# ElijahHyndman/PAPTeam_OpticalFlow

Hardware: AMD Instinct MI355X
Metric: Mpix/s per frame-pair (fixed SOR iters) at 1920x1080; max-abs d(u,v) vs ref (higher is better)
Workload: dtype f64

## Files before the change

papteam_opticalflow_amd/csrc/api.hip:

```cpp
#include <algorithm>
#include <chrono>
#include <cmath>
#include <cstdio>
#include <cstdlib>
#include <cstring>
#include <mutex>
#include <random>
#include <thread>

#include "common.h"
#include "flow_internal.h"

namespace papof {

namespace {
thread_local std::string g_last_error;
}

void set_last_error(const char* what, hipError_t e, const char* file, int line) {
    char buf[512];
    std::snprintf(buf, sizeof buf, "%s failed: %s (%s:%d)", what, hipGetErrorString(e), file, line);
    g_last_error = buf;
}
const char* last_error() { return g_last_error.c_str(); }
void set_last_error_text(const std::string& text) { g_last_error = text; }

static double wall() {
    return std::chrono::duration<double>(std::chrono::steady_clock::now().time_since_epoch()).count();
}

size_t arena_bytes_for(int H, int W, int C, int levels, int n_sor_max, double ratio) {
    const size_t np = (size_t)H * W;
    const int fc = (C == 3) ? 5 : (C == 1 ? 3 : C);
    size_t per_level = 0;
    {
        std::vector<Level> L;
        std::vector<PyrPlan> plan;
        if (levels >= 1 && pyramid_plan(H, W, ratio, levels, L, plan) == PAPOF_OK)
            for (const Level& l : L) per_level += ((size_t)l.w * l.h * fc * sizeof(double) + 256) * 3;
    }
    size_t sor_cells = 0, sor_cells_d = 0;
    skew_capacity(H, W, n_sor_max, sor_cells, sor_cells_d);
    size_t planes = 0;
    planes += (size_t)2 * C * 5;
    if (levels > 8) planes += (size_t)2 * C * levels;
    planes += (size_t)2 * C + 2 * C;
    planes += (size_t)7 * fc;
    planes += 8;
    planes += (size_t)3 * C + C;
    planes += (size_t)3 * fc;
    size_t bytes = planes * np * sizeof(double);
    bytes += 3 * (sor_cells + 2 * kLanes) * 16 + (sor_cells_d + 2 * kLanes) * 16 + 10 * np * sizeof(double);
    bytes += per_level + np * fc * sizeof(double);
    bytes += 8 * (std::min<size_t>(kTinyMaxCells, np) * sizeof(double) + 256);
    bytes += (size_t)64 * 4096;
    return bytes;
}

static size_t sor_scratch_bytes(int H, int W, int n_sor) {
    size_t cells = 0, cells_d = 0;
    skew_capacity(H, W, n_sor, cells, cells_d);
    return 4 * (cells + 128) * 16 + (cells_d + 128) * 16;
}

int ensure_arena(papof_handle* h, size_t bytes) {
    if (bytes <= h->arena.cap) return PAPOF_OK;
    PAPOF_HIP(hipStreamSynchronize(h->stream));
    if (h->arena.base) PAPOF_HIP(hipFree(h->arena.base));
    h->arena.base = nullptr;
    h->arena.cap = 0;
    void* p = nullptr;
    hipError_t e = hipMalloc(&p, bytes);
    if (e != hipSuccess) {
        set_last_error("hipMalloc(arena)", e, __FILE__, __LINE__);
        return PAPOF_ENOMEM;
    }
    h->arena.base = static_cast<char*>(p);
    h->arena.cap = bytes;
    return PAPOF_OK;
}

int check_params(const papof_params& P, int levels) {
    if (levels < 1) return PAPOF_EINVAL;
    if (P.n_inner < 1) return PAPOF_EINVAL;
    if (P.n_outer + 0 < 1 || P.n_sor < 1 || P.n_outer_per_level < 0 || P.n_sor_per_level < 0) return PAPOF_EINVAL;
    if (P.sor_mode < PAPOF_SOR_EXACT || P.sor_mode > PAPOF_SOR_JACOBI) return PAPOF_EINVAL;
    if (!(P.alpha > 0) || !(P.omega > 0)) return PAPOF_EINVAL;
    if (P.interpolation != PAPOF_INTERP_BILINEAR && P.interpolation != PAPOF_INTERP_BICUBIC) return PAPOF_EINVAL;
    if (P.noise_model != PAPOF_NOISE_LAPLACIAN && P.noise_model != PAPOF_NOISE_GMIXTURE) return PAPOF_EINVAL;
    return PAPOF_OK;
}

int pyramid_plan(int H, int W, double ratio, int nlev, std::vector<Level>& L, std::vector<PyrPlan>& plan) {
    ratio = effective_ratio(ratio);
    const double base_sigma = 1 / ratio - 1;
    const int n = (int)(std::log(0.25) / std::log(ratio));
    const double n_sigma = base_sigma * n;
    L.assign(nlev, Level{});
    plan.assign(nlev, PyrPlan{});
    L[0].w = W;
    L[0].h = H;
    for (int i = 1; i < nlev; i++) {
        PyrPlan p;
        if (i <= n) {
            p.src_level = 0;
            p.sigma = base_sigma * i;
            p.fsize = (int)(p.sigma * 3);
            p.rate = std::pow(ratio, i);
        } else {
            p.src_level = i - n;
            p.sigma = n_sigma;
            p.fsize = (int)(n_sigma * 3);
            p.rate = (double)std::pow(ratio, i) * W / L[i - n].w;
        }
        p.sw = L[p.src_level].w;
        p.sh = L[p.src_level].h;
        if (p.fsize > kMaxFsize) return PAPOF_EINVAL;
        L[i].w = (int)((double)p.sw * p.rate);
        L[i].h = (int)((double)p.sh * p.rate);
        if (L[i].w < 1 || L[i].h < 1) return PAPOF_EINVAL;
        plan[i] = p;
    }
    return PAPOF_OK;
}

papof_params params_or_default(const papof_params* params) {
    papof_params P;
    if (params)
        P = *params;
    else
        papof_default_params(&P);
    return P;
}

int call_plan(int H, int W, int C, int levels, const papof_params& P, CallPlan& cp) {
    PAPOF_TRY(check_params(P, levels));
    cp.ratio = effective_ratio(P.ratio);
    cp.levels = levels;
    cp.fc = feature_channels(C);
    PAPOF_TRY(pyramid_plan(H, W, P.ratio, levels, cp.L, cp.plan));
    cp.n_sor.resize(levels);
    cp.n_outer.resize(levels);
    for (int k = 0; k < levels; k++) {
        cp.n_sor[k] = CallPlan::n_sor_at(P, k);
        cp.n_outer[k] = CallPlan::n_outer_at(P, k);
    }
    cp.n_sor_max = cp.n_sor[levels - 1];
    cp.slots = CallPlan::slots_for(P, levels);
    cp.from_level0 = true;
    for (int i = 1; i < levels; i++) cp.from_level0 = cp.from_level0 && cp.plan[i].src_level == 0;
    return PAPOF_OK;
}

int lap_next_epoch(papof_handle* h, hipStream_t stream) {
    if (++h->lap_epoch >= kLapNone) {
        if (h->lap_flags_dev) PAPOF_HIP(hipMemsetAsync(h->lap_flags_dev, 0, kLapFlagWords * sizeof(unsigned), stream));
        h->lap_epoch = 1u;
    }
    return PAPOF_OK;
}

int fork_prep(papof_handle* h, int levels, bool overlap) {
    while (h->sync_events.size() < (size_t)levels + 2) {
        hipEvent_t e;
        PAPOF_HIP(hipEventCreateWithFlags(&e, hipEventDisableTiming));
        h->sync_events.push_back(e);
    }
    if (overlap) {
        PAPOF_HIP(hipEventRecord(h->sync_events[levels + 1], h->stream));
        PAPOF_HIP(hipStreamWaitEvent(h->prep_stream, h->sync_events[levels + 1], 0));
    }
    return PAPOF_OK;
}

int smooth_and_resize(papof_handle* h, const double* src, double* dst, double* tmp_a, double* tmp_b, const PyrPlan& p, int C,
                      int dh, int dw) {
    const Taps g = gaussian_taps(p.sigma, p.fsize);
    if (g.fsize == 0 && g.t[0] == 1.0) return resize(h, src, dst, p.sh, p.sw, C, dh, dw, p.rate, p.rate, false, 0.0);
    PAPOF_TRY(filter_hv(h, src, tmp_b, tmp_a, p.sh, p.sw, C, g, g));
    return resize(h, tmp_b, dst, p.sh, p.sw, C, dh, dw, p.rate, p.rate, false, 0.0);
}

int reduce_init(papof_handle* h, const papof_tensor* a, const papof_tensor* b, int pairs_a, int pairs_b, int H, int W,
                const std::vector<Level>& L, const std::vector<PyrPlan>& plan, double ratio, double* X, double* Y, double* T,
                size_t t_planes, double*& out) {
    const size_t np0 = (size_t)H * W;
    const int planes = 2 * (pairs_a + pairs_b), levels = (int)L.size();
    double* const parts[2] = {X, X + (size_t)pairs_a * 2 * np0};
    const papof_tensor* const src[2] = {a, b};
    const int n[2] = {pairs_a, pairs_b};
    for (int i = 0; i < 2; i++) {
        if (n[i] == 0) continue;
        if (src[i])
            PAPOF_TRY(ingest_frames(h, *src[i], nullptr, parts[i], H, W, 2, n[i]));
        else
            PAPOF_HIP(hipMemsetAsync(parts[i], 0, (size_t)n[i] * 2 * np0 * sizeof(double), h->stream));
    }
    PAPOF_TRY(init_sanitize(h, X, (size_t)planes * np0));
    out = X;
    if (levels == 1) return PAPOF_OK;
    std::vector<int> chain;
    for (int i = levels - 1; i > 0; i = plan[i].src_level) chain.insert(chain.begin(), i);
    double s = 1.0;
    for (int i = 1; i < levels; i++) s *= ratio;
    double *cur = X, *other = Y;
    for (const int i : chain) {
        const PyrPlan& p = plan[i];
        const bool last = i == levels - 1;
        const Taps g = gaussian_taps(p.sigma, p.fsize);
        if (g.fsize == 0 && g.t[0] == 1.0) {
            PAPOF_TRY(resize(h, cur, other, p.sh, p.sw, planes, L[i].h, L[i].w, p.rate, p.rate, last, last ? s : 0.0));
            std::swap(cur, other);
            continue;
        }
        const size_t ns = (size_t)p.sw * p.sh;
        const int chunk = filter_hv_needs_tmp(g, g) ? (int)std::min<size_t>((size_t)planes, t_planes * np0 / ns) : planes;
        if (chunk < 1) return PAPOF_EINVAL;
        for (int c0 = 0; c0 < planes; c0 += chunk)
            PAPOF_TRY(filter_hv(h, cur + c0 * ns, other + c0 * ns, T, p.sh, p.sw, std::min(chunk, planes - c0), g, g));
        PAPOF_TRY(resize(h, other, cur, p.sh, p.sw, planes, L[i].h, L[i].w, p.rate, p.rate, last, last ? s : 0.0));
    }
    out = cur;
    return PAPOF_OK;
}

int build_pyramid(papof_handle* h, const std::vector<Level>& L, const std::vector<PyrPlan>& plan, int C, bool second,
                  double* tmp_a, double* tmp_b) {
    for (size_t i = 1; i < L.size(); i++) {
        const PyrPlan& p = plan[i];
        const double* src = second ? L[p.src_level].p2 : L[p.src_level].p1;
        double* dst = second ? L[i].p2 : L[i].p1;
        PAPOF_TRY(smooth_and_resize(h, src, dst, tmp_a, tmp_b, p, C, L[i].h, L[i].w));
    }
    return PAPOF_OK;
}

struct SolveBuffers {
    double *im1s, *tmp, *blend, *imdt, *phi;
    SorPlanes sp;
    SorPlanes sp_tiny{};
    double *bgx = nullptr, *bgy = nullptr, *bgxy = nullptr;
    double *gm = nullptr, *gm_scratch = nullptr;
};

int alloc_solve_buffers(Arena& A, int H, int W, int fc, int mode, int n_sor_cap, SolveBuffers& B) {
    const size_t np = (size_t)H * W;
    B.im1s = A.f64(np * fc);
    B.tmp = A.f64(np * fc);
    B.blend = A.f64(np * fc);
    B.imdt = A.f64(np * fc);
    B.phi = A.f64(np);
    PAPOF_TRY(sor_alloc_planes(A, H, W, mode, n_sor_cap, B.sp));
    if (mode == PAPOF_SOR_EXACT)
        PAPOF_TRY(sor_alloc_tiny_planes(A, std::min<size_t>(kTinyMaxCells, (size_t)H * W), B.sp_tiny));
    return A.overflow ? PAPOF_ENOMEM : PAPOF_OK;
}

int alloc_branch_buffers(papof_handle* h, Arena& A, int H, int W, int fc, int interpolation, int noise_model,
                         SolveBuffers& B) {
    const size_t np = (size_t)H * W;
    if (interpolation == PAPOF_INTERP_BICUBIC) {
        B.bgx = A.f64(np * fc);
        B.bgy = A.f64(np * fc);
        B.bgxy = A.f64(np * fc);
    }
    if (noise_model == PAPOF_NOISE_GMIXTURE) {
        B.gm = A.f64(5 * 8);
        B.gm_scratch = A.f64((size_t)gm_scratch_doubles());
        if (A.overflow || fc > 8) return fc > 8 ? PAPOF_EINVAL : PAPOF_ENOMEM;
        double init[40];
        for (int k = 0; k < fc; k++) {
            init[k] = 0.95;
            init[fc + k] = 0.05;
            init[2 * fc + k] = 0.5;
            init[3 * fc + k] = 0.05 * 0.05;
            init[4 * fc + k] = 0.5 * 0.5;
        }
        PAPOF_HIP(hipMemcpyAsync(B.gm, init, sizeof(double) * 5 * fc, hipMemcpyHostToDevice, h->stream));
        PAPOF_HIP(hipStreamSynchronize(h->stream));
    }
    return A.overflow ? PAPOF_ENOMEM : PAPOF_OK;
}

struct LapGuard {
    bool on = false;
    bool exact = false;
    bool collect = false;
    bool nz_known = false;
    unsigned* flags = nullptr;
    double* lap = nullptr;
    double* scratch = nullptr;
    unsigned epoch = 0;
    int slot = 0;
    std::vector<int> slot_level, slot_channels;
    unsigned* wit(int s) const { return on && collect && s >= 0 && s < kLapMaxSlots ? flags + lap_wit_word(s) : nullptr; }
    unsigned* nz(int level) const { return on && collect && nz_known ? flags + lap_nz_word(level) : nullptr; }
    const double* guard() const { return on && exact ? lap : nullptr; }
    int unknown(const unsigned* host_flags) const {
        if (!on || !collect) return 0;
        if (slot > kLapMaxSlots) return 1;
        int n = 0;
        for (int s = 0; s + 1 < slot; s++)
            for (int c = 0; c < slot_channels[s]; c++) {
                const unsigned nz = host_flags[lap_nz_word(slot_level[s]) + c];
                const bool proven = lap_proven(host_flags[lap_wit_word(s) + c], epoch, nz_known, nz, nz);
                n += !proven;
                if (!proven && std::getenv("PAPOF_LAP_TRACE"))
                    std::fprintf(stderr, "[lap guard] no proof: slot %d of %d, level %d, channel %d\n", s, slot, slot_level[s], c);
            }
        return n;
    }
};

struct LevelSolve {
    SolveBuffers& B;
    const double *f1 = nullptr, *f2 = nullptr;
    double* warp = nullptr;
    int H = 0, W = 0, fc = 0;
    double alpha = 0, omega = 0;
    int n_outer = 0, n_inner = 0, n_sor = 0, mode = PAPOF_SOR_EXACT;
    const double* im1s_ready = nullptr;
    bool final_warp = true;
    const SolveCounters* counters = nullptr;
    double *out_u = nullptr, *out_v = nullptr;
    bool fold_warp = false;
    LapGuard* lg = nullptr;
    int level = 0;
};

static int marked_solve(papof_handle* h, PhaseClock& clk, unsigned* prog, SorPlanes& SP, const LevelSolve& s) {
    h->sor_mark = [](void* c, int on) {
        static_cast<PhaseClock*>(c)->phase(on ? PAPOF_T_PHASE5_SOR : PAPOF_T_PHASE6_UPDATE);
    };
    h->sor_mark_ctx = &clk;
    h->sor_prog_next = prog;
    const int rc = sor_solve(h, SP, s.H, s.W, s.alpha, s.omega, s.n_sor, s.mode);
    h->sor_prog_next = nullptr;
    h->sor_mark = nullptr;
    h->sor_mark_ctx = nullptr;
    return rc;
}

int smooth_flow(papof_handle* h, const LevelSolve& s, PhaseClock& clk, double*& u, double*& v, double*& ua, double*& va) {
    SolveBuffers& B = s.B;
    const Taps g = smooth5_taps();
    int solve_idx = 0;
    const bool tiny = s.mode == PAPOF_SOR_EXACT && B.sp_tiny.phi && sor_tiny_fits(h, s.H, s.W, s.n_sor);
    SorPlanes& SP = tiny ? B.sp_tiny : B.sp;
    const double* im1s = s.im1s_ready;
    if (!im1s) {
        clk.phase(PAPOF_T_PHASE1_GENERATE);
        PAPOF_TRY(filter_hv(h, s.f1, B.im1s, B.tmp, s.H, s.W, s.fc, g, g));
        im1s = B.im1s;
    }
    const char* const fused_sw = std::getenv("PAPOF_FUSED_SYSTEM");
    const bool fused_env = !(fused_sw && fused_sw[0] == '0');
    const bool fused_system = fused_env && s.fold_warp && s.n_inner == 1 && !B.gm && (s.fc == 5 || s.fc == 3) &&
                              !(s.lg && s.lg->guard()) && !(s.lg && s.lg->on && lap_one_block_level(s.H, s.W));
    for (int count = 0; count < s.n_outer; count++) {
        clk.phase(fused_system ? kTimerFused : (int)PAPOF_T_PHASE1_GENERATE);
        if (fused_system)
            PAPOF_TRY(flow_system(h, s.f1, s.f2, u, v, im1s, s.H, s.W, s.fc, s.alpha, s.omega, SP,
                                  s.lg && count > 0 ? s.lg->wit(s.lg->slot - 1) : nullptr));
        else if (s.fold_warp)
            PAPOF_TRY(warp_smooth_blend(h, s.f1, s.f2, u, v, im1s, B.blend, B.imdt, s.H, s.W, s.fc,
                                        s.lg && count > 0 && !B.gm ? s.lg->wit(s.lg->slot - 1) : nullptr,
                                        B.phi));
        else
            PAPOF_TRY(smooth_hv_blend(h, s.warp, im1s, B.blend, B.imdt, s.H, s.W, s.fc));
        for (int hh = 0; hh < s.n_inner; hh++) {
            const SorPlanes* prev = hh == 0 ? nullptr : &SP;
            if ((count == 0 && !s.fold_warp) || hh > 0) {
                clk.phase(PAPOF_T_PHASE2_DERIVATIVES);
                PAPOF_TRY(compute_phi(h, u, v, prev, B.phi, s.H, s.W));
            }
            if (!fused_system) clk.phase(PAPOF_T_PHASE4_LINEARSYSTEM);
            if (!fused_system)
                PAPOF_TRY(assemble_system(h, B.blend, B.imdt, B.phi, u, v, s.H, s.W, s.fc, s.alpha, s.omega, SP, nullptr, nullptr,
                                          prev, nullptr, B.gm, s.lg ? s.lg->guard() : nullptr));
            PAPOF_TRY(marked_solve(h, clk, s.counters ? s.counters->solve(h, s.level, (size_t)solve_idx) : nullptr, SP, s));
            solve_idx++;
        }
        double* const phi_next = count + 1 < s.n_outer && !s.fold_warp ? B.phi : nullptr;
        const bool rewarp = !s.fold_warp && !B.bgx && (s.final_warp || count + 1 < s.n_outer || B.gm);
        const bool wit_later = s.fold_warp && count + 1 < s.n_outer;
        const bool wit_small = s.fold_warp && !wit_later && lap_one_block_level(s.H, s.W);
        unsigned* const wit = s.lg && !B.gm && !B.bgx && !wit_later && !wit_small ? s.lg->wit(s.lg->slot) : nullptr;
        const bool to_caller = s.out_u && s.out_v && count + 1 == s.n_outer;
        PAPOF_TRY(update_warp_phi(h, SP, u, v, to_caller ? s.out_u : ua, to_caller ? s.out_v : va, s.f1, s.f2, s.warp, phi_next,
                                  s.H, s.W, s.fc, rewarp, 0, -1, wit));
        if (to_caller) {
            u = s.out_u;
            v = s.out_v;
        } else {
            std::swap(u, ua);
            std::swap(v, va);
        }
        if (B.bgx)
            PAPOF_TRY(bicubic_warp(h, s.f1, s.f2, B.bgx, B.bgy, B.bgxy, u, v, s.warp, s.H, s.W, s.fc, nullptr, true, true));
        if (s.lg && s.lg->on && !B.gm && wit_small && s.lg->wit(s.lg->slot))
            PAPOF_TRY(lap_small_check(h, s.f1, s.f2, u, v, s.H, s.W, s.fc, s.lg->wit(s.lg->slot)));
        if (s.lg && s.lg->on && !B.gm) {
            s.lg->slot_level.push_back(s.level);
            s.lg->slot_channels.push_back(s.fc);
            s.lg->slot++;
            if (s.lg->exact) {
                if (B.bgx)
                    PAPOF_TRY(est_laplacian_noise(h, s.f1, s.warp, nullptr, nullptr, s.H, s.W, s.fc, s.lg->lap, s.lg->scratch));
                else
                    PAPOF_TRY(est_laplacian_noise(h, s.f1, s.f2, u, v, s.H, s.W, s.fc, s.lg->lap, s.lg->scratch));
            }
        }
        if (B.gm) PAPOF_TRY(est_gaussian_mixture(h, s.f1, s.warp, s.H, s.W, s.fc, B.gm, B.gm_scratch));
    }
    clk.phase(-1);
    return PAPOF_OK;
}

int feature_channels(int C) { return C == 3 ? 5 : (C == 1 ? 3 : C); }

struct FrameIn {
    const void* d;
    bool u8;
    bool planar = false;
};
int load_frame(papof_handle* h, const FrameIn& f, double* planar, int H, int W, int C) {
    if (f.planar) {
        PAPOF_HIP(hipMemcpyAsync(planar, f.d, (size_t)H * W * C * sizeof(double), hipMemcpyDeviceToDevice, h->stream));
        return PAPOF_OK;
    }
    if (f.u8) return hwc_u8_to_planar(h, static_cast<const unsigned char*>(f.d), planar, H, W, C);
    return hwc_to_planar(h, static_cast<const double*>(f.d), planar, H, W, C);
}

enum SeqOp { kPair, kSeqPrime, kSeqNext };

bool seq_matches(const papof_handle* h, int H, int W, int C, int levels, double ratio, size_t need) {
    const papof_handle::Seq& q = h->seq;
    return q.valid && q.h == H && q.w == W && q.c == C && q.levels == levels && q.ratio == ratio &&
           q.arena_base == h->arena.base && need <= h->arena.cap;
}

struct FlowPass {
    papof_handle* h;
    const FrameIn &fa, &fb;
    SeqOp op;
    int H, W, C;
    const papof_params& P;
    double *d_vx, *d_vy, *d_warp;
    LapGuard* lg;
    const papof_tensor* init;
    CallPlan cp;
    int slot1 = 0;
    double *tmp_a = nullptr, *tmp_b = nullptr;
    std::vector<double*> F1, F2, S1;
    double *gx = nullptr, *gy = nullptr, *gxy = nullptr;
    double *prep_tmp = nullptr, *warp = nullptr;
    double *u = nullptr, *v = nullptr, *u2 = nullptr, *v2 = nullptr;
    SolveBuffers B;
    bool exact = false;
    SolveCounters counters;
    bool overlap = false;
    bool hostio = false;
    hipStream_t main_stream = nullptr, prep = nullptr;
    PhaseClock clk, pclk, total;
};

static void keep_seq(const FlowPass& S, int slot) {
    S.h->seq = {.valid = true, .h = S.H, .w = S.W, .c = S.C, .levels = S.cp.levels, .slot = slot, .ratio = S.cp.ratio,
                .arena_base = S.h->arena.base};
}

static void start_clocks(FlowPass& S) {
    papof_handle* h = S.h;
    S.clk = S.pclk = S.total = PhaseClock{h, true};
    S.clk.only_sor = S.pclk.only_sor = (!h->phase_events && S.P.phase_timing == 0) || S.P.phase_timing == 2;
    h->sor_launches = 0;
    h->sor_log.clear();
    S.clk.stamps = true;
    h->stamps_used = 0;
    h->next_stamp = nullptr;
    h->stamp_stream = h->stream;
    S.total.phase(PAPOF_T_TOTAL);
}

static int carve_pyramids(FlowPass& S) {
    Arena& A = S.h->arena;
    for (Level& l : S.cp.L) {
        double* slot[2];
        slot[0] = A.f64((size_t)l.w * l.h * S.C);
        slot[1] = A.f64((size_t)l.w * l.h * S.C);
        l.p1 = slot[S.slot1];
        l.p2 = slot[S.slot1 ^ 1];
    }
    const size_t np0 = (size_t)S.H * S.W;
    S.tmp_a = A.f64(np0 * S.C);
    S.tmp_b = A.f64(np0 * S.C);
    return A.overflow ? PAPOF_ENOMEM : PAPOF_OK;
}

static int carve_buffers(FlowPass& S) {
    papof_handle* h = S.h;
    Arena& A = h->arena;
    const CallPlan& cp = S.cp;
    const int levels = cp.levels, fc = cp.fc;
    const size_t np0 = (size_t)S.H * S.W;
    S.F1.resize(levels);
    S.F2.resize(levels);
    S.S1.resize(levels);
    for (int k = 0; k < levels; k++) {
        const size_t n = (size_t)cp.L[k].w * cp.L[k].h * fc;
        S.F1[k] = A.f64(n);
        S.F2[k] = A.f64(n);
        S.S1[k] = A.f64(n);
    }
    S.prep_tmp = A.f64(np0 * fc);
    S.gx = A.f64(np0 * S.C);
    S.gy = A.f64(np0 * S.C);
    S.gxy = A.f64(np0 * S.C);
    S.warp = A.f64(np0 * fc);
    S.u = A.f64(2 * np0);
    S.v = S.u ? S.u + np0 : nullptr;
    S.u2 = A.f64(2 * np0);
    S.v2 = S.u2 ? S.u2 + np0 : nullptr;
    PAPOF_TRY(alloc_solve_buffers(A, S.H, S.W, fc, S.P.sor_mode, cp.n_sor_max, S.B));
    PAPOF_TRY(alloc_branch_buffers(h, A, S.H, S.W, fc, S.P.interpolation, S.P.noise_model, S.B));
    S.exact = S.P.sor_mode == PAPOF_SOR_EXACT;
    if (S.exact) {
        S.counters = SolveCounters(cp, [&](int k) { return sor_counters_words(cp.L[k].h, cp.L[k].w, cp.n_sor[k]); },
                                   (size_t)S.P.n_inner);
        PAPOF_TRY(sor_counters_ensure(h, S.counters.total));
    }
    return PAPOF_OK;
}

static bool prep_kept(const FlowPass& S, int second) { return second == 0 && S.op == kSeqNext; }
static int prep_build_level(FlowPass& S, int i, int second) {
    if (i == 0 || prep_kept(S, second)) return PAPOF_OK;
    const std::vector<Level>& L = S.cp.L;
    const PyrPlan& q = S.cp.plan[i];
    const double* src = second ? L[q.src_level].p2 : L[q.src_level].p1;
    return smooth_and_resize(S.h, src, second ? L[i].p2 : L[i].p1, S.tmp_a, S.tmp_b, q, S.C, L[i].h, L[i].w);
}
static int prep_level_ready(FlowPass& S, int k) {
    S.pclk.phase(-1);
    if (S.overlap) PAPOF_HIP(hipEventRecord(S.h->sync_events[k], S.prep));
    return PAPOF_OK;
}
static int prep_frames(FlowPass& S, int first, int last, bool chained, bool smooth, bool ready) {
    const std::vector<Level>& L = S.cp.L;
    const int levels = S.cp.levels;
    const Taps g5 = smooth5_taps();
    S.pclk.phase(PAPOF_T_CONSTRUCTION);
    for (int second = first; second < last; second++)
        if (!prep_kept(S, second)) PAPOF_TRY(load_frame(S.h, second ? S.fb : S.fa, second ? L[0].p2 : L[0].p1, S.H, S.W, S.C));
    for (int i = 1; chained && i < levels; i++)
        for (int second = first; second < last; second++) PAPOF_TRY(prep_build_level(S, i, second));
    for (int k = levels - 1; k >= 0; k--) {
        if (!chained) {
            S.pclk.phase(PAPOF_T_CONSTRUCTION);
            for (int second = first; second < last; second++) PAPOF_TRY(prep_build_level(S, k, second));
        }
        S.pclk.phase(PAPOF_T_ALLOCATION);
        for (int second = first; second < last; second++)
            PAPOF_TRY(im2feature(S.h, second ? L[k].p2 : L[k].p1, second ? S.F2[k] : S.F1[k], L[k].h, L[k].w, S.C,
                                 S.lg ? S.lg->nz(k) : nullptr));
        if (smooth) {
            S.pclk.phase(PAPOF_T_PHASE1_GENERATE);
            PAPOF_TRY(filter_hv(S.h, S.F1[k], S.S1[k], S.prep_tmp, L[k].h, L[k].w, S.cp.fc, g5, g5));
        }
        if (ready) PAPOF_TRY(prep_level_ready(S, k));
    }
    return PAPOF_OK;
}
static int prep_final_planes(FlowPass& S) {
    S.pclk.phase(PAPOF_T_POSTPROCESSING);
    PAPOF_TRY(central3_planes(S.h, S.cp.L[0].p2, S.gx, S.gy, S.gxy, S.H, S.W, S.C));
    return prep_level_ready(S, S.cp.levels);
}
static int prep_upload(FlowPass& S, const void* host, const FrameIn& f, int event) {
    papof_handle* h = S.h;
    if (!host) return PAPOF_OK;
    PAPOF_HIP(hipMemcpyAsync(const_cast<void*>(f.d), host, h->hostio.nb_in, hipMemcpyHostToDevice, h->copy_stream));
    PAPOF_HIP(hipEventRecord(h->copy_events[event], h->copy_stream));
    PAPOF_HIP(hipStreamWaitEvent(S.prep, h->copy_events[event], 0));
    return PAPOF_OK;
}

static int prepare(FlowPass& S) {
    StreamSwap on_prep(S.h, S.prep);
    const bool chained = !S.cp.from_level0;
    S.pclk.phase(PAPOF_T_ALLOCATION);
    if (S.exact && !sor_counters_clear(S.h, 0, S.counters.total)) return PAPOF_EDEVICE;
    if (!S.hostio) {
        PAPOF_TRY(prep_frames(S, 0, 2, chained, true, true));
    } else {
        PAPOF_TRY(prep_upload(S, S.h->hostio.im1, S.fa, 0));
        PAPOF_TRY(prep_frames(S, 0, 1, true, true, false));
        S.pclk.phase(-1);
        PAPOF_TRY(prep_upload(S, S.h->hostio.im2, S.fb, 1));
        PAPOF_TRY(prep_frames(S, 1, 2, chained, false, true));
    }
    return prep_final_planes(S);
}

static int fork_and_prepare(FlowPass& S) {
    papof_handle* h = S.h;
    const papof_handle::HostIO& io = h->hostio;
    S.overlap = h->overlap_prep && S.P.phase_timing != 1 && h->prep_stream != nullptr;
    S.main_stream = h->stream;
    S.prep = S.overlap ? h->prep_stream : h->stream;
    S.hostio = io.active && S.overlap && h->copy_stream && h->copy_events.size() >= 8;
    if (io.active && !S.hostio) {
        if (io.im1) PAPOF_HIP(hipMemcpyAsync(const_cast<void*>(S.fa.d), io.im1, io.nb_in, hipMemcpyHostToDevice, S.main_stream));
        if (io.im2) PAPOF_HIP(hipMemcpyAsync(const_cast<void*>(S.fb.d), io.im2, io.nb_in, hipMemcpyHostToDevice, S.main_stream));
    }
    PAPOF_TRY(fork_prep(h, S.cp.levels, S.overlap));
    const int rc = prepare(S);
    if (rc != PAPOF_OK && S.overlap) hipStreamSynchronize(S.prep);
    return rc;
}

static int enter_level(FlowPass& S, int k, int pw, int ph, bool fold_warp) {
    papof_handle* h = S.h;
    const int lw = S.cp.L[k].w, lh = S.cp.L[k].h, fc = S.cp.fc;
    const size_t np = (size_t)lw * lh;
    const double *f1 = S.F1[k], *f2 = S.F2[k];
    SolveBuffers& B = S.B;
    const bool coarsest = k == S.cp.levels - 1;
    if (coarsest && S.init) {
        double* r = nullptr;
        PAPOF_TRY(reduce_init(h, S.init, nullptr, 1, 0, S.H, S.W, S.cp.L, S.cp.plan, S.cp.ratio, S.u, S.u2, S.warp, (size_t)fc, r));
        if (r != S.u) std::swap(S.u, S.u2);
    } else if (coarsest) {
        PAPOF_HIP(hipMemsetAsync(S.u, 0, 2 * np * sizeof(double), h->stream));
        if (!fold_warp) PAPOF_HIP(hipMemcpyAsync(S.warp, f2, np * fc * sizeof(double), hipMemcpyDeviceToDevice, h->stream));
    } else {
        PAPOF_TRY(resize(h, S.u, S.u2, ph, pw, 2, lh, lw, (double)lw / pw, (double)lh / ph, true, 1 / S.cp.ratio));
        std::swap(S.u, S.u2);
    }
    S.v = S.u + np;
    S.v2 = S.u2 + np;
    if (B.bgx) PAPOF_TRY(central3_planes(h, f2, B.bgx, B.bgy, B.bgxy, lh, lw, fc));
    if (coarsest && !S.init) return PAPOF_OK;
    if (B.bgx)
        PAPOF_TRY(bicubic_warp(h, f1, f2, B.bgx, B.bgy, B.bgxy, S.u, S.v, S.warp, lh, lw, fc, nullptr, true, false));
    else if (!fold_warp)
        PAPOF_TRY(warp_bilinear(h, f1, f2, S.u, S.v, S.warp, lh, lw, fc));
    return PAPOF_OK;
}

static int solve_levels(FlowPass& S) {
    papof_handle* h = S.h;
    const CallPlan& cp = S.cp;
    LapGuard* const lg = S.lg;
    if (lg && lg->guard())
        PAPOF_HIP(hipMemcpyAsync(lg->lap, h->lap_init_dev, 8 * sizeof(double), hipMemcpyDeviceToDevice, S.main_stream));
    int pw = 0, ph = 0;
    for (int k = cp.levels - 1; k >= 0; k--) {
        const int lw = cp.L[k].w, lh = cp.L[k].h;
        S.clk.phase(-1);
        if (S.overlap) PAPOF_HIP(hipStreamWaitEvent(S.main_stream, h->sync_events[k], 0));
        S.clk.phase(PAPOF_T_ALLOCATION);
        const bool tiny_k = S.exact && sor_tiny_fits(h, lh, lw, cp.n_sor[k]);
        if (!tiny_k) PAPOF_TRY(sor_bind(h, S.B.sp, lh, lw, cp.n_sor[k]));
        const LevelSolve s{.B = S.B, .f1 = S.F1[k], .f2 = S.F2[k], .warp = S.warp, .H = lh, .W = lw, .fc = cp.fc,
                           .alpha = S.P.alpha, .omega = S.P.omega, .n_outer = cp.n_outer[k], .n_inner = S.P.n_inner,
                           .n_sor = cp.n_sor[k], .mode = S.P.sor_mode, .im1s_ready = S.S1[k], .final_warp = false,
                           .counters = S.exact ? &S.counters : nullptr, .out_u = k == 0 ? S.d_vx : nullptr,
                           .out_v = k == 0 ? S.d_vy : nullptr, .fold_warp = !S.B.bgx && !S.B.gm, .lg = lg, .level = k};
        PAPOF_TRY(enter_level(S, k, pw, ph, s.fold_warp));
        if (!tiny_k) PAPOF_TRY(sor_reset_planes(h, S.B.sp));
        PAPOF_TRY(smooth_flow(h, s, S.clk, S.u, S.v, S.u2, S.v2));
        pw = lw;
        ph = lh;
    }
    return PAPOF_OK;
}

static int final_warp(FlowPass& S) {
    papof_handle* h = S.h;
    papof_handle::HostIO& io = h->hostio;
    const int H = S.H, W = S.W, C = S.C, levels = S.cp.levels;
    const size_t np0 = (size_t)H * W;
    const Level& l0 = S.cp.L[0];
    S.clk.phase(-1);
    if (S.overlap) PAPOF_HIP(hipStreamWaitEvent(S.main_stream, h->sync_events[levels], 0));
    S.clk.phase(PAPOF_T_POSTPROCESSING);
    if (S.hostio && io.early_out && S.u == S.d_vx && S.v == S.d_vy) {
        hipStream_t const cs = h->copy_stream;
        PAPOF_HIP(hipEventRecord(h->copy_events[2], S.main_stream));
        PAPOF_HIP(hipStreamWaitEvent(cs, h->copy_events[2], 0));
        PAPOF_HIP(hipMemcpyAsync(io.vx, S.d_vx, io.nb_flow, hipMemcpyDeviceToHost, cs));
        PAPOF_HIP(hipMemcpyAsync(io.vy, S.d_vy, io.nb_flow, hipMemcpyDeviceToHost, cs));
        constexpr int kChunks = 4;
        for (int q = 0; q < kChunks; q++) {
            const Rect rc{0, (int)((long long)H * q / kChunks), W, (int)((long long)H * (q + 1) / kChunks)};
            if (rc.empty()) continue;
            PAPOF_TRY(bicubic_warp(h, l0.p1, l0.p2, S.gx, S.gy, S.gxy, S.u, S.v, S.d_warp, H, W, C, &rc));
            PAPOF_HIP(hipEventRecord(h->copy_events[3 + q], S.main_stream));
            PAPOF_HIP(hipStreamWaitEvent(cs, h->copy_events[3 + q], 0));
            const size_t off = (size_t)rc.y0 * W * C, cnt = (size_t)rc.h() * W * C;
            PAPOF_HIP(hipMemcpyAsync(io.warp + off, S.d_warp + off, cnt * sizeof(double), hipMemcpyDeviceToHost, cs));
        }
        io.out_issued = true;
        return PAPOF_OK;
    }
    PAPOF_TRY(bicubic_warp(h, l0.p1, l0.p2, S.gx, S.gy, S.gxy, S.u, S.v, S.d_warp, H, W, C));
    if (S.u != S.d_vx) PAPOF_HIP(hipMemcpyAsync(S.d_vx, S.u, np0 * sizeof(double), hipMemcpyDeviceToDevice, h->stream));
    if (S.v != S.d_vy) PAPOF_HIP(hipMemcpyAsync(S.d_vy, S.v, np0 * sizeof(double), hipMemcpyDeviceToDevice, h->stream));
    return PAPOF_OK;
}

static int fetch_flags_and_stamps(FlowPass& S) {
    papof_handle* h = S.h;
    const LapGuard* lg = S.lg;
    h->stamps_fetched = 0;
    const bool flags = lg && lg->on && lg->collect;
    const size_t first = flags ? lap_wit_word(std::min(lg->slot, kLapMaxSlots) - 1) : kLapFlagWords;
    const size_t bytes = (kLapFlagWords - first) * sizeof(unsigned) + (size_t)h->stamps_used * sizeof(unsigned long long);
    if (bytes > 0)
        PAPOF_HIP(hipMemcpyAsync(h->lap_flags_host + first, h->lap_flags_dev + first, bytes, hipMemcpyDeviceToHost, h->stream));
    h->stamps_fetched = h->stamps_used;
    return PAPOF_OK;
}

static void report_timers(double* tm) {
    {
        constexpr double kPsiShare = 0.3;
        const double fused = tm[PAPOF_T_PHASE4_LINEARSYSTEM];
        tm[PAPOF_T_PHASE3_PSIDATA] += kPsiShare * fused;
        tm[PAPOF_T_PHASE4_LINEARSYSTEM] = fused - kPsiShare * fused;
    }
    {
        constexpr double kPhiShare = 0.04;
        const double fused = tm[PAPOF_T_PHASE1_GENERATE];
        tm[PAPOF_T_PHASE2_DERIVATIVES] += kPhiShare * fused;
        tm[PAPOF_T_PHASE1_GENERATE] = fused - kPhiShare * fused;
    }
    {
        const double f = tm[kTimerFused];
        tm[PAPOF_T_PHASE1_GENERATE] += 0.51 * f;
        tm[PAPOF_T_PHASE2_DERIVATIVES] += 0.02 * f;
        tm[PAPOF_T_PHASE3_PSIDATA] += 0.14 * f;
        tm[PAPOF_T_PHASE4_LINEARSYSTEM] += f - 0.51 * f - 0.02 * f - 0.14 * f;
    }
}

int flow_pass(papof_handle* h, const FrameIn& fa, const FrameIn& fb, SeqOp op, int H, int W, int C, int levels,
              const papof_params& P, double* d_vx, double* d_vy, double* d_warp, double* timing, LapGuard* lg,
              const papof_tensor* init = nullptr) {
    const double t_entry = wall();
    FlowPass S{h, fa, fb, op, H, W, C, P, d_vx, d_vy, d_warp, lg, init};
    PAPOF_TRY(call_plan(H, W, C, levels, P, S.cp));
    const size_t need = arena_bytes_for(H, W, C, levels, S.cp.n_sor_max, P.ratio);
    if (op == kSeqNext && !seq_matches(h, H, W, C, levels, S.cp.ratio, need)) {
        g_last_error = "sequence push does not continue the primed sequence (shape, levels, ratio or arena changed)";
        return PAPOF_EINVAL;
    }
    S.slot1 = op == kSeqNext ? h->seq.slot : 0;
    h->seq.valid = false;
    PAPOF_TRY(ensure_arena(h, need));
    h->arena.off = 0;
    h->arena.overflow = false;
    h->events_used = 0;
    double tm[PAPOF_N_TIMERS + 1];
    std::memset(tm, 0, sizeof tm);
    start_clocks(S);
    PAPOF_TRY(carve_pyramids(S));
    if (op == kSeqPrime) {
        PAPOF_TRY(load_frame(h, fa, S.cp.L[0].p1, H, W, C));
        PAPOF_TRY(build_pyramid(h, S.cp.L, S.cp.plan, C, false, S.tmp_a, S.tmp_b));
        PAPOF_HIP(hipStreamSynchronize(h->stream));
        keep_seq(S, S.slot1);
        if (timing) std::memset(timing, 0, PAPOF_N_TIMERS * sizeof(double));
        return PAPOF_OK;
    }
    PAPOF_TRY(carve_buffers(S));
    PAPOF_TRY(fork_and_prepare(S));
    int rc_main = solve_levels(S);
    if (rc_main == PAPOF_OK) rc_main = final_warp(S);
    if (rc_main != PAPOF_OK) {
        hipStreamSynchronize(S.main_stream);
        if (S.overlap) hipStreamSynchronize(S.prep);
        return rc_main;
    }
    S.clk.phase(-1);
    PAPOF_TRY(stamp_only(h));
    S.total.phase(-1);
    PAPOF_TRY(fetch_flags_and_stamps(S));
    const double t_enqueued = wall();
    PAPOF_HIP(hipStreamSynchronize(h->stream));
    h->host_enqueue_sec = t_enqueued - t_entry;
    h->host_wait_sec = wall() - t_enqueued;
    h->next_stamp = nullptr;
    if (S.exact) PAPOF_TRY(sor_check(h));
    if (S.clk.err != PAPOF_OK || S.pclk.err != PAPOF_OK || S.total.err != PAPOF_OK) return PAPOF_EDEVICE;
    S.clk.collect(tm);
    S.pclk.collect(tm);
    S.total.collect(tm);
    if (S.clk.sor_span_sec.size() == h->sor_log.size())
        for (size_t i = 0; i < h->sor_log.size(); i++) h->sor_log[i].sec = S.clk.sor_span_sec[i];
    report_timers(tm);
    if (timing) std::memcpy(timing, tm, PAPOF_N_TIMERS * sizeof(double));
    if (op == kSeqNext) keep_seq(S, S.slot1 ^ 1);
    return PAPOF_OK;
}

int flow_device(papof_handle* h, const FrameIn& fa, const FrameIn& fb, SeqOp op, int H, int W, int C, int levels,
                const papof_params& P, double* d_vx, double* d_vy, double* d_warp, double* timing,
                const papof_tensor* init = nullptr) {
    LapGuard lg;
    const int fc = feature_channels(C);
    lg.on = h->lap_guard && op != kSeqPrime && P.noise_model == PAPOF_NOISE_LAPLACIAN && fc <= 8 && levels >= 1 &&
            h->lap_flags_dev != nullptr;
    if (!lg.on) return flow_pass(h, fa, fb, op, H, W, C, levels, P, d_vx, d_vy, d_warp, timing, nullptr, init);
    lg.flags = h->lap_flags_dev;
    lg.lap = h->lap_dev;
    lg.scratch = h->lap_scratch_dev;
    lg.nz_known = (C == 1 || C == 3) && (size_t)levels * 8 <= (size_t)kLapNzWords;
    const bool always_exact = P.interpolation == PAPOF_INTERP_BICUBIC;
    lg.collect = !always_exact;
    lg.exact = always_exact || h->lap_exact;
    const papof_handle::Seq seq0 = h->seq;
    double first_pass_total = 0.0;
    for (int pass = 0; pass < 2; pass++) {
        PAPOF_TRY(lap_next_epoch(h, h->stream));
        lg.epoch = h->lap_epoch;
        lg.slot = 0;
        lg.slot_level.clear();
        lg.slot_channels.clear();
        PAPOF_TRY(flow_pass(h, fa, fb, op, H, W, C, levels, P, d_vx, d_vy, d_warp, timing, &lg, init));
        if (pass == 1 && timing) timing[PAPOF_T_TOTAL] += first_pass_total;
        if (!lg.collect) return PAPOF_OK;
        const int unknown = lg.unknown(h->lap_flags_host);
        if (lg.exact) {
            if (pass == 0) h->lap_exact_calls++;
            h->lap_exact = unknown > 0;
            return PAPOF_OK;
        }
        if (unknown == 0) return PAPOF_OK;
        h->lap_reruns++;
        lg.exact = true;
        if (timing) first_pass_total = timing[PAPOF_T_TOTAL];
        if (h->copy_stream) PAPOF_HIP(hipStreamSynchronize(h->copy_stream));
        h->seq = seq0;
        h->hostio.im1 = nullptr;
        h->hostio.im2 = nullptr;
    }
    return PAPOF_OK;
}

int flow_device_planar(papof_handle* h, const double* f1, const double* f2, int H, int W, int C, int levels,
                       const papof_params& P, double* d_vx, double* d_vy, double* d_warp, double* timing,
                       const papof_tensor* init) {
    FrameIn a{f1, false}, b{f2, false};
    a.planar = b.planar = true;
    return flow_device(h, a, b, kPair, H, W, C, levels, P, d_vx, d_vy, d_warp, timing, init);
}

}
// ... 653 lines not shown
    PAPOF_TRY(S.down_planar(sp.b1, rhs1, height, width, 1));
    return S.down_planar(sp.b2, rhs2, height, width, 1);
}

int papof_stage_laplacian(papof_handle* h, const double* in, const double* weight, int height, int width,
                          double* out) {
    if (!h || !in || !weight || !out || height < 1 || width < 1) return PAPOF_EINVAL;
    Scope S(h, img_bytes(height, width, 1, 6));
    PAPOF_TRY(S.rc);
    double* a = S.up_planar(in, height, width, 1);
    double* w = S.up_planar(weight, height, width, 1);
    double* o = S.dev((size_t)height * width);
    PAPOF_TRY(S.rc);
    PAPOF_TRY(laplacian(h, a, w, o, height, width));
    return S.down_planar(o, out, height, width, 1);
}

namespace {
int alloc_sor_planes(Scope& S, int H, int W, int mode, int n_sor, SorPlanes& sp) {
    if (mode == PAPOF_SOR_EXACT && sor_tiny_fits(S.h, H, W, n_sor)) {
        const int rc_t = sor_alloc_tiny_planes(S.h->arena, (size_t)H * W, sp);
        if (rc_t != PAPOF_OK) S.rc = rc_t;
        return S.rc;
    }
    int rc = sor_alloc_planes(S.h->arena, H, W, mode, n_sor, sp);
    if (rc == PAPOF_OK) rc = sor_bind(S.h, sp, H, W, n_sor);
    if (rc != PAPOF_OK) S.rc = rc;
    return S.rc;
}
}

int papof_stage_sor(papof_handle* h, const double* phi, const double* imdxy, const double* imdx2,
                    const double* imdy2, const double* rhs1, const double* rhs2, int height, int width,
                    double alpha, double omega, int n_sor, int sor_mode, double* du, double* dv) {
    if (!h || !phi || !imdxy || !imdx2 || !imdy2 || !rhs1 || !rhs2 || !du || !dv || height < 1 || width < 1 ||
        n_sor < 1 || sor_mode < PAPOF_SOR_EXACT || sor_mode > PAPOF_SOR_JACOBI)
        return PAPOF_EINVAL;
    const size_t np = (size_t)height * width;
    Scope S(h, img_bytes(height, width, 1, 16) + sor_scratch_bytes(height, width, n_sor) +
                   12 * (size_t)height * width * sizeof(double));
    PAPOF_TRY(S.rc);
    double* p = S.up_planar(phi, height, width, 1);
    double* xy = S.up_planar(imdxy, height, width, 1);
    double* x2 = S.up_planar(imdx2, height, width, 1);
    double* y2 = S.up_planar(imdy2, height, width, 1);
    double* r1 = S.up_planar(rhs1, height, width, 1);
    double* r2 = S.up_planar(rhs2, height, width, 1);
    double *ou = S.dev(np), *ov = S.dev(np);
    SorPlanes sp{};
    PAPOF_TRY(alloc_sor_planes(S, height, width, sor_mode, n_sor, sp));
    PAPOF_TRY(sor_reset_planes(h, sp));
    PAPOF_TRY(sor_prep(h, p, xy, x2, y2, r1, r2, height, width, alpha, omega, sp));
    PAPOF_TRY(sor_solve(h, sp, height, width, alpha, omega, n_sor, sor_mode));
    PAPOF_TRY(sor_unpack(h, sp, ou, ov, height, width));
    PAPOF_TRY(S.down_planar(ou, du, height, width, 1));
    PAPOF_TRY(S.down_planar(ov, dv, height, width, 1));
    if (sor_mode == PAPOF_SOR_EXACT) PAPOF_TRY(sor_check(h));
    return PAPOF_OK;
}

int papof_stage_smoothflow(papof_handle* h, const double* im1, const double* im2, double* warp, double* u,
                           double* v, int height, int width, int c, double alpha, int n_outer, int n_inner,
                           int n_sor, double omega, int sor_mode) {
    return papof_stage_smoothflow_ex(h, im1, im2, warp, u, v, height, width, c, alpha, n_outer, n_inner, n_sor, omega,
                                     sor_mode, PAPOF_INTERP_BILINEAR, PAPOF_NOISE_LAPLACIAN, nullptr);
}

int papof_stage_smoothflow_ex(papof_handle* h, const double* im1, const double* im2, double* warp, double* u,
                              double* v, int height, int width, int c, double alpha, int n_outer, int n_inner,
                              int n_sor, double omega, int sor_mode, int interpolation, int noise_model, double* gm) {
    if (!h || !im1 || !im2 || !warp || !u || !v || height < 1 || width < 1 || c < 1 || n_outer < 1 || n_sor < 1 ||
        sor_mode < PAPOF_SOR_EXACT || sor_mode > PAPOF_SOR_JACOBI)
        return PAPOF_EINVAL;
    if (n_inner < 1) return PAPOF_EINVAL;
    if (interpolation < 0 || interpolation > 1 || noise_model < 0 || noise_model > 1) return PAPOF_EINVAL;
    Scope S(h, img_bytes(height, width, c, 16) + img_bytes(height, width, 1, 8) +
                   sor_scratch_bytes(height, width, n_sor) +
                   12 * (size_t)height * width * sizeof(double) + (1 << 20));
    PAPOF_TRY(S.rc);
    double* f1 = S.up_planar(im1, height, width, c);
    double* f2 = S.up_planar(im2, height, width, c);
    double* w = S.up_planar(warp, height, width, c);
    double* du = S.up_planar(u, height, width, 1);
    double* dv = S.up_planar(v, height, width, 1);
    double* du_alt = S.dev((size_t)height * width);
    double* dv_alt = S.dev((size_t)height * width);
    PAPOF_TRY(S.rc);
    SolveBuffers B;
    PAPOF_TRY(alloc_solve_buffers(h->arena, height, width, c, sor_mode, n_sor, B));
    PAPOF_TRY(alloc_branch_buffers(h, h->arena, height, width, c, interpolation, noise_model, B));
    if (B.gm && gm) PAPOF_HIP(hipMemcpyAsync(B.gm, gm, sizeof(double) * 5 * c, hipMemcpyHostToDevice, h->stream));
    if (B.bgx) PAPOF_TRY(central3_planes(h, f2, B.bgx, B.bgy, B.bgxy, height, width, c));
    PAPOF_TRY(sor_bind(h, B.sp, height, width, n_sor));
    PAPOF_TRY(sor_reset_planes(h, B.sp));
    PhaseClock clk{h, false};
    LapGuard lg;
    lg.on = h->lap_guard && noise_model == PAPOF_NOISE_LAPLACIAN && c <= 8 && h->lap_dev != nullptr;
    lg.exact = true;
    lg.lap = h->lap_dev;
    lg.scratch = h->lap_scratch_dev;
    if (lg.on) PAPOF_HIP(hipMemcpyAsync(lg.lap, h->lap_init_dev, 8 * sizeof(double), hipMemcpyDeviceToDevice, h->stream));
    const LevelSolve s{.B = B, .f1 = f1, .f2 = f2, .warp = w, .H = height, .W = width, .fc = c, .alpha = alpha, .omega = omega,
                       .n_outer = n_outer, .n_inner = n_inner, .n_sor = n_sor, .mode = sor_mode, .lg = &lg};
    PAPOF_TRY(smooth_flow(h, s, clk, du, dv, du_alt, dv_alt));
    PAPOF_TRY(S.down_planar(w, warp, height, width, c));
    PAPOF_TRY(S.down_planar(du, u, height, width, 1));
    PAPOF_TRY(S.down_planar(dv, v, height, width, 1));
    if (B.gm && gm) {
        PAPOF_HIP(hipMemcpyAsync(gm, B.gm, sizeof(double) * 5 * c, hipMemcpyDeviceToHost, h->stream));
        PAPOF_HIP(hipStreamSynchronize(h->stream));
    }
    if (sor_mode == PAPOF_SOR_EXACT) PAPOF_TRY(sor_check(h));
    return PAPOF_OK;
}

int papof_stage_est_gaussian_mixture(papof_handle* h, const double* im1, const double* im2, int height, int width,
                                     int c, double* gm) {
    if (!h || !im1 || !im2 || !gm || height < 1 || width < 1 || c < 1 || c > 8) return PAPOF_EINVAL;
    Scope S(h, img_bytes(height, width, c, 6) + (1 << 20));
    PAPOF_TRY(S.rc);
    double* a = S.up_planar(im1, height, width, c);
    double* b = S.up_planar(im2, height, width, c);
    double* g = S.dev(40);
    double* scratch = S.dev((size_t)gm_scratch_doubles());
    PAPOF_TRY(S.rc);
    PAPOF_HIP(hipMemcpyAsync(g, gm, sizeof(double) * 5 * c, hipMemcpyHostToDevice, h->stream));
    PAPOF_TRY(est_gaussian_mixture(h, a, b, height, width, c, g, scratch));
    PAPOF_HIP(hipMemcpyAsync(gm, g, sizeof(double) * 5 * c, hipMemcpyDeviceToHost, h->stream));
    PAPOF_HIP(hipStreamSynchronize(h->stream));
    return PAPOF_OK;
}

int papof_pyramid_levels_for_min_width(int width, double ratio, int min_width, int* levels) {
    if (width < 1 || min_width < 1 || !levels) return PAPOF_EINVAL;
    ratio = effective_ratio(ratio);
    *levels = (int)(std::log((double)min_width / width) / std::log(ratio));
    return PAPOF_OK;
}

int papof_sor_tiny_shape(int height, int width, int* cells_per_tile, int* waves) {
    if (height < 1 || width < 1 || !cells_per_tile || !waves) return PAPOF_EINVAL;
    sor_tiny_shape(height, width, cells_per_tile, waves);
    return PAPOF_OK;
}

int papof_stage_bicubic_warp(papof_handle* h, const double* im1, const double* im2, const double* vx,
                             const double* vy, int height, int width, int c, double* out) {
    return papof_stage_bicubic_warp_ex(h, im1, im2, vx, vy, height, width, c, 1, out);
}

int papof_stage_bicubic_warp_ex(papof_handle* h, const double* im1, const double* im2, const double* vx,
                                const double* vy, int height, int width, int c, int clamp, double* out) {
    if (!h || !im1 || !im2 || !vx || !vy || !out || height < 1 || width < 1 || c < 1) return PAPOF_EINVAL;
    Scope S(h, img_bytes(height, width, c, 10) + img_bytes(height, width, 1, 4));
    PAPOF_TRY(S.rc);
    const size_t n = (size_t)height * width * c;
    double* a = S.up_planar(im1, height, width, c);
    double* b = S.up_planar(im2, height, width, c);
    double* fx = S.up_planar(vx, height, width, 1);
    double* fy = S.up_planar(vy, height, width, 1);
    double *gx = S.dev(n), *gy = S.dev(n), *gxy = S.dev(n), *o = S.dev(n);
    PAPOF_TRY(S.rc);
    PAPOF_TRY(central3_planes(h, b, gx, gy, gxy, height, width, c));
    PAPOF_TRY(bicubic_warp(h, a, b, gx, gy, gxy, fx, fy, o, height, width, c, nullptr, false, clamp != 0));
    PAPOF_HIP(hipMemcpyAsync(out, o, n * sizeof(double), hipMemcpyDeviceToHost, h->stream));
    PAPOF_HIP(hipStreamSynchronize(h->stream));
    return PAPOF_OK;
}

int papof_flow_quantize16(papof_handle* h, const double* vx, const double* vy, int height, int width,
                          unsigned short* out) {
    if (!h || !vx || !vy || !out || height < 1 || width < 1) return PAPOF_EINVAL;
    const size_t n = (size_t)height * width;
    Scope S(h, n * (2 * sizeof(double) + 2 * sizeof(unsigned short)) + 4096);
    PAPOF_TRY(S.rc);
    double* a = S.up_planar(vx, height, width, 1);
    double* b = S.up_planar(vy, height, width, 1);
    unsigned short* q = reinterpret_cast<unsigned short*>(S.dev((n * 2 * sizeof(unsigned short) + 7) / 8));
    PAPOF_TRY(S.rc);
    PAPOF_TRY(flow_quantize16(h, a, b, q, n));
    PAPOF_HIP(hipMemcpyAsync(out, q, n * 2 * sizeof(unsigned short), hipMemcpyDeviceToHost, h->stream));
    PAPOF_HIP(hipStreamSynchronize(h->stream));
    return PAPOF_OK;
}

int papof_flow_dequantize16(papof_handle* h, const unsigned short* q, int height, int width, double* vx,
                            double* vy) {
    if (!h || !q || !vx || !vy || height < 1 || width < 1) return PAPOF_EINVAL;
    const size_t n = (size_t)height * width;
    Scope S(h, n * (2 * sizeof(double) + 2 * sizeof(unsigned short)) + 4096);
    PAPOF_TRY(S.rc);
    unsigned short* dq = reinterpret_cast<unsigned short*>(S.dev((n * 2 * sizeof(unsigned short) + 7) / 8));
    double* a = S.dev(n);
    double* b = S.dev(n);
    PAPOF_TRY(S.rc);
    PAPOF_HIP(hipMemcpyAsync(dq, q, n * 2 * sizeof(unsigned short), hipMemcpyHostToDevice, h->stream));
    PAPOF_TRY(flow_dequantize16(h, dq, a, b, n));
    PAPOF_HIP(hipMemcpyAsync(vx, a, n * sizeof(double), hipMemcpyDeviceToHost, h->stream));
    PAPOF_HIP(hipMemcpyAsync(vy, b, n * sizeof(double), hipMemcpyDeviceToHost, h->stream));
    PAPOF_HIP(hipStreamSynchronize(h->stream));
    return PAPOF_OK;
}

int papof_flow_to_bgr(papof_handle* h, const double* vx, const double* vy, int height, int width,
                      unsigned char* bgr) {
    if (!h || !vx || !vy || !bgr || height < 1 || width < 1) return PAPOF_EINVAL;
    const size_t n = (size_t)height * width;
    Scope S(h, n * (2 * sizeof(double) + 3) + 16384);
    PAPOF_TRY(S.rc);
    double* a = S.up_planar(vx, height, width, 1);
    double* b = S.up_planar(vy, height, width, 1);
    double* partial = S.dev(512);
    unsigned char* out = reinterpret_cast<unsigned char*>(S.dev((n * 3 + 7) / 8));
    PAPOF_TRY(S.rc);
    PAPOF_TRY(flow_to_bgr(h, a, b, n, partial, out));
    PAPOF_HIP(hipMemcpyAsync(bgr, out, n * 3, hipMemcpyDeviceToHost, h->stream));
    PAPOF_HIP(hipStreamSynchronize(h->stream));
    return PAPOF_OK;
}

int papof_sor_plan(papof_handle* h, int height, int width, int n_sor, int sor_mode, int* launches, int* depth) {
    return sor_plan(h, height, width, n_sor, sor_mode, launches, depth);
}

int papof_last_sor_stats(papof_handle* h, int* launches, double* strip_streams_sec) {
    if (!h) return PAPOF_EINVAL;
    if (launches) *launches = h->sor_launches;
    if (strip_streams_sec) *strip_streams_sec = 0.0;
    return PAPOF_OK;
}

int papof_lap_guard_stats(papof_handle* h, int out[4]) {
    if (!h || !out) return PAPOF_EINVAL;
    out[0] = h->lap_reruns;
    out[1] = h->lap_exact_calls;
    out[2] = h->lap_exact ? 1 : 0;
    out[3] = h->lap_guard ? 1 : 0;
    return PAPOF_OK;
}

int papof_last_host_times(papof_handle* h, double out[3]) {
    if (!h || !out) return PAPOF_EINVAL;
    out[0] = h->host_enqueue_sec;
    out[1] = h->host_wait_sec;
    out[2] = 0.0;
    return PAPOF_OK;
}

int papof_last_sor_solves(papof_handle* h, int cap, int* n, int* info, double* sec) {
    if (!h || !n) return PAPOF_EINVAL;
    *n = (int)h->sor_log.size();
    for (int i = 0; i < *n && i < cap; i++) {
        const papof_handle::SorSolveLog& e = h->sor_log[i];
        if (info) {
            int* o = info + (size_t)i * 6;
            o[0] = e.H;
            o[1] = e.W;
            o[2] = e.n_sor;
            o[3] = e.kind;
            o[4] = e.depth;
            o[5] = e.launches;
        }
        if (sec) sec[i] = e.sec;
    }
    return PAPOF_OK;
}

int papof_test_sor_strips(papof_handle* h, int height, int width, int n_sor, int split_band, int reps, int delay_us,
                          long long* mismatches, int* bands) {
    if (!h || !mismatches) return PAPOF_EINVAL;
    const size_t np = (size_t)height * width;
    Scope S(h, img_bytes(height, width, 1, 16) + sor_scratch_bytes(height, width, n_sor) +
                   12 * (size_t)height * width * sizeof(double));
    PAPOF_TRY(S.rc);
    std::vector<double> host(np * 6);
    std::mt19937_64 rng(2);
    auto fill = [&](size_t k, double lo, double hi) {
        std::uniform_real_distribution<double> d(lo, hi);
        for (size_t i = 0; i < np; i++) host[k * np + i] = d(rng);
    };
    fill(0, 0.5, 50.0);
    fill(1, -0.02, 0.02);
    fill(2, 0.0, 0.05);
    fill(3, 0.0, 0.05);
    fill(4, -0.01, 0.01);
    fill(5, -0.01, 0.01);
    double* planes[6];
    for (int k = 0; k < 6; k++) planes[k] = S.up_planar(host.data() + k * np, height, width, 1);
    SorPlanes sp{};
    PAPOF_TRY(alloc_sor_planes(S, height, width, PAPOF_SOR_EXACT, n_sor, sp));
    PAPOF_TRY(sor_reset_planes(h, sp));
    PAPOF_TRY(sor_prep(h, planes[0], planes[1], planes[2], planes[3], planes[4], planes[5], height, width, 0.012, 1.8, sp));
    if (bands) *bands = sp.sd.nb;
    const size_t cells = sp.sd.nd;
    std::vector<double> want(cells * 2), got(cells * 2);
    PAPOF_TRY(sor_solve(h, sp, height, width, 0.012, 1.8, n_sor, PAPOF_SOR_EXACT));
    PAPOF_HIP(hipStreamSynchronize(h->stream));
    PAPOF_TRY(sor_check(h));
    PAPOF_HIP(hipMemcpy(want.data(), sp.du, cells * 16, hipMemcpyDeviceToHost));
    *mismatches = 0;
    if (!sor_strips_supported(h, sp, n_sor) || split_band < 1 || split_band >= sp.sd.nb) return PAPOF_EINVAL;
    struct Owned {
        hipStream_t top = nullptr;
        hipEvent_t ev = nullptr;
        ~Owned() {
            if (top) {
                hipStreamSynchronize(top);
                hipStreamDestroy(top);
            }
            if (ev) hipEventDestroy(ev);
        }
    } own;
    PAPOF_HIP(hipStreamCreateWithFlags(&own.top, hipStreamNonBlocking));
    PAPOF_HIP(hipEventCreateWithFlags(&own.ev, hipEventDisableTiming));
    hipStream_t const main_stream = h->stream, top = own.top;
    hipEvent_t const ev = own.ev;
    for (int r = 0; r < reps; r++) {
// ... 172 lines not shown
```

papteam_opticalflow_amd/csrc/common.h:

```cpp
#pragma once
#include <cstdlib>

#include <hip/hip_runtime.h>

#include <algorithm>
#include <cmath>
#include <cstddef>
#include <cstdint>
#include <initializer_list>
#include <string>
#include <vector>

#include "../../include/papof.h"

namespace papof {

constexpr int kLanes = 64;
constexpr int kMaxFsize = 8;

struct Rect {
    int x0, y0, x1, y1;
    __host__ __device__ bool empty() const { return x1 <= x0 || y1 <= y0; }
    __host__ __device__ int w() const { return x1 - x0; }
    __host__ __device__ int h() const { return y1 - y0; }
// ... 114 lines not shown
        d.hp = (d.rt + kBandRows * d.nb + 2 + 7) / 8 * 8;
        d.npos = d.qt + d.ns + 2 * kSorMaxDepth + 2 + kBandRows * (d.nb - 1) + 2;
        d.dpar = d.group == 1 ? ((n_sor - 1) & 1) : (((n_sor + d.group - 1) / d.group - 1) & 1);
        d.koff = n_sor - 1;
        d.poff = 1;
        d.nh = d.group == 1 ? 0 : (size_t)n_sor * d.nb * d.npos_d;
    }
    d.n = (size_t)d.npos * d.hp;
    d.nd = (size_t)2 * d.npos_d * d.nb * kLanes;
    return d;
}
inline void skew_capacity(int h, int w, int n_sor, size_t& cells, size_t& cells_d) {
    const SkewDims a = skew_dims(h, w, n_sor, 2), b = skew_dims(h, w, n_sor, 1, 2);
    cells = a.n > b.n ? a.n : b.n;
    cells_d = (a.nd + a.nh) > (b.nd + b.nh) ? (a.nd + a.nh) : (b.nd + b.nh);
}

struct SorPlanes {
    double *phi, *xy, *a1, *a2, *b1, *b2;
    double *du, *dv;
    double *du2, *dv2;
    bool skew;
    SkewDims sd;
    size_t cap_cells, cap_cells_d;
};

}

struct papof_handle {
    int device = 0;
    hipStream_t stream = nullptr;
    papof::Arena arena;
    unsigned* sync_words = nullptr;
    size_t sync_cap = 0;
    std::vector<hipEvent_t> events;
    size_t events_used = 0;
    int cu_count = 0;
    double* stage_dev = nullptr;
    size_t stage_dev_bytes = 0;
    double* tensor_scratch = nullptr;
    size_t tensor_scratch_bytes = 0;
    hipEvent_t entry_event = nullptr;
    unsigned* init_flag_dev = nullptr;
    bool use_dpp = false;
    int sor_depth = 0;
    unsigned long long* sor_dbg = nullptr;
    void (*sor_mark)(void*, int) = nullptr;
    void* sor_mark_ctx = nullptr;
    int sor_fuse = 0;
    int sor_group = 0;
    int rb_depth = 0;
    int rb_shape = 0;
    int sor_tiny = 1;
    int sor_resident = 0;
    int sor_skip_dead = 1;
    unsigned* sor_prog_next = nullptr;
    int sor_launches = 0;
    struct SorSolveLog {
        int H, W, n_sor, kind, depth, launches;
        double sec;
    };
    std::vector<SorSolveLog> sor_log;
    hipStream_t prep_stream = nullptr;
    unsigned* lap_flags_dev = nullptr;
    unsigned* lap_flags_host = nullptr;
    double* lap_dev = nullptr;
    double* lap_init_dev = nullptr;
    double* lap_scratch_dev = nullptr;
    bool lap_guard = true;
    bool lap_exact = false;
    unsigned lap_epoch = 0;
    int lap_reruns = 0, lap_exact_calls = 0;
    long long batch_chains = 0, batch_chain_pairs = 0, batch_singles = 0, batch_reruns = 0;
    double host_enqueue_sec = 0.0, host_wait_sec = 0.0;
    struct HostIO {
        bool active = false;
        const void *im1 = nullptr, *im2 = nullptr;
        size_t nb_in = 0;
        double *vx = nullptr, *vy = nullptr, *warp = nullptr;
        size_t nb_flow = 0, nb_img = 0;
        bool early_out = false;
        bool out_issued = false;
    } hostio;
    hipStream_t copy_stream = nullptr;
    std::vector<hipEvent_t> copy_events;
    std::vector<hipEvent_t> sync_events;
    bool overlap_prep = true;
    unsigned long long* stamps_dev = nullptr;
    unsigned long long* stamps = nullptr;
    int stamps_cap = 0, stamps_used = 0, stamps_fetched = 0;
    unsigned long long* next_stamp = nullptr;
    hipStream_t stamp_stream = nullptr;
    bool phase_events = true;
    int sor_xcd_affine = 1;
    struct Seq {
        bool valid = false;
        int h = 0, w = 0, c = 0, levels = 0, slot = 0;
        double ratio = 0;
        const char* arena_base = nullptr;
    } seq;
};

namespace papof {

inline unsigned long long* take_stamp(papof_handle* h) {
    if (h->stamp_stream && h->stream != h->stamp_stream) return nullptr;
    unsigned long long* s = h->next_stamp;
    h->next_stamp = nullptr;
    return s;
}
int stamp_only(papof_handle* h);

inline bool described(const papof_tensor* t, std::initializer_list<int> dtypes, std::initializer_list<int> axes, bool positive) {
    if (!t || !t->data || std::find(dtypes.begin(), dtypes.end(), t->dtype) == dtypes.end()) return false;
    for (int i : axes)
        if (t->stride[i] < 0 || (positive && t->stride[i] == 0)) return false;
    return true;
}
constexpr std::initializer_list<int> kImageDtypes = {PAPOF_DTYPE_U8, PAPOF_DTYPE_F32, PAPOF_DTYPE_F64};
constexpr std::initializer_list<int> kFlowDtypes = {PAPOF_DTYPE_F32, PAPOF_DTYPE_F64};
inline bool in_frames(const papof_tensor* t) { return described(t, kImageDtypes, {0, 1, 2, 3}, false); }
inline bool out_frames(const papof_tensor* t) { return described(t, kImageDtypes, {0, 1, 2, 3}, true); }
inline bool in_flow(const papof_tensor* t) { return described(t, kFlowDtypes, {0, 1, 2, 3}, false); }
inline bool out_flow(const papof_tensor* t) { return described(t, kFlowDtypes, {0, 1, 2, 3}, true); }
inline bool in_flow_pair(const papof_tensor* fw, const papof_tensor* bw) { return in_flow(fw) && in_flow(bw); }
inline bool opt_in_mask(const papof_tensor* t) { return !t || described(t, {PAPOF_DTYPE_U8}, {0, 1, 2}, false); }
inline bool opt_out_mask(const papof_tensor* t) { return !t || described(t, {PAPOF_DTYPE_U8}, {0, 1, 2}, true); }
inline bool opt_in_plane(const papof_tensor* t) { return !t || described(t, kFlowDtypes, {0, 1, 2}, false); }
inline bool opt_out_plane(const papof_tensor* t) { return !t || described(t, kFlowDtypes, {0, 1, 2}, true); }
inline bool valid_alphas(double a1, double a2) { return std::isfinite(a1) && std::isfinite(a2) && a1 >= 0 && a2 >= 0; }
inline long long dtype_bytes(int dtype) { return dtype == PAPOF_DTYPE_U8 ? 1 : dtype == PAPOF_DTYPE_F32 ? 4 : 8; }

int hwc_to_planar(papof_handle* h, const double* hwc, double* planar, int H, int W, int C, int frames = 1);
int hwc_u8_to_planar(papof_handle* h, const unsigned char* hwc, double* planar, int H, int W, int C, int frames = 1);
int planar_to_hwc(papof_handle* h, const double* planar, double* hwc, int H, int W, int C);
int ingest_frames(papof_handle* h, const papof_tensor& a, const papof_tensor* b, double* planar, int H, int W, int C,
                  int frames);
int emit_outputs(papof_handle* h, const double* src, const papof_tensor& dst, bool comp_major, int H, int W, int K, int pairs);
int init_check(papof_handle* h, const papof_tensor& t, int pairs, int H, int W, unsigned* flag);
int init_sanitize(papof_handle* h, double* planar, size_t n);
int fb_check(papof_handle* h, hipStream_t st, const papof_tensor& fw, const papof_tensor& bw, const papof_tensor& mask,
             int pairs, int H, int W, double a1, double a2);
int filter_h(papof_handle* h, const double* src, double* dst, int H, int W, int planes, const Taps& f,
             const Rect* rc = nullptr);
int filter_v(papof_handle* h, const double* src, double* dst, int H, int W, int planes, const Taps& f,
             const Rect* rc = nullptr);
int filter_hv(papof_handle* h, const double* src, double* dst, double* tmp, int H, int W, int planes, const Taps& fh,
              const Taps& fv);
bool filter_hv_needs_tmp(const Taps& fh, const Taps& fv);
int resize(papof_handle* h, const double* src, double* dst, int sh, int sw, int planes, int dh, int dw, double xr,
           double yr, bool use_post, double post, const Rect* rc = nullptr);
int im2feature(papof_handle* h, const double* im, double* feat, int H, int W, int C, unsigned* nz = nullptr, int frames = 1,
               size_t nz_stride = 0);
int central3_planes(papof_handle* h, const double* src, double* gx, double* gy, double* gxy, int H, int W, int planes);
int warp_bilinear(papof_handle* h, const double* im1, const double* im2, const double* vx, const double* vy,
                  double* out, int H, int W, int planes, const Rect* rc = nullptr);
int smooth_v_blend(papof_handle* h, const double* tmp, const double* im1s, double* blend, double* imdt, int H,
                   int W, int planes, const Rect* rc = nullptr);
int smooth_hv_blend(papof_handle* h, const double* warp, const double* im1s, double* blend, double* imdt, int H,
                    int W, int planes, int row0 = 0, int row1 = -1);
int warp_smooth_blend(papof_handle* h, const double* im1, const double* im2, const double* u, const double* v,
                      const double* im1s, double* blend, double* imdt, int H, int W, int planes, unsigned* wit = nullptr,
                      double* phi_out = nullptr);
int compute_phi(papof_handle* h, const double* u, const double* v, const SorPlanes* prev, double* phi, int H, int W,
                const Rect* rc = nullptr);
int assemble_system(papof_handle* h, const double* blend, const double* imdt, const double* phi, const double* u,
                    const double* v, int H, int W, int planes, double alpha, double omega, const SorPlanes& out,
                    double* opt_imdx2, double* opt_imdy2, const SorPlanes* prev, const Rect* rc = nullptr,
                    const double* gm = nullptr, const double* lap = nullptr);
int flow_system(papof_handle* h, const double* im1, const double* im2, const double* u, const double* v, const double* im1s,
                int H, int W, int planes, double alpha, double omega, const SorPlanes& out, unsigned* wit = nullptr,
                int row0 = 0, int row1 = -1,
                int batch = 1, const BatchK* bk = nullptr);
int lap_scratch_doubles();
int lap_rows_check(papof_handle* h, const double* im1, const double* im2, const double* u, const double* v, int H, int W,
                   int C, int r0, int r1, unsigned* wit, unsigned* val, unsigned mark);
bool lap_one_block_level(int H, int W);
int lap_small_check(papof_handle* h, const double* im1, const double* im2, const double* u, const double* v, int H, int W,
                    int C, unsigned* wit, int batch = 1, const BatchK* bk = nullptr);
int est_laplacian_noise(papof_handle* h, const double* im1, const double* im2, const double* u, const double* v, int H,
                        int W, int C, double* lap, double* scratch);
int gm_scratch_doubles();
int est_gaussian_mixture(papof_handle* h, const double* im1, const double* im2, int H, int W, int C, double* gm,
                         double* scratch);
int laplacian(papof_handle* h, const double* in, const double* weight, double* out, int H, int W);
int bicubic_warp(papof_handle* h, const double* im1, const double* im2, const double* gx, const double* gy,
                 const double* gxy, const double* vx, const double* vy, double* out_hwc, int H, int W, int C,
                 const Rect* rc = nullptr, bool planar_out = false, bool clamp = true, int batch = 1, const BatchK* bk = nullptr);
int flow_quantize16(papof_handle* h, const double* vx, const double* vy, unsigned short* q, size_t n);
int flow_dequantize16(papof_handle* h, const unsigned short* q, double* vx, double* vy, size_t n);
int flow_to_bgr(papof_handle* h, const double* vx, const double* vy, size_t n, double* partial, unsigned char* bgr);
int update_warp_phi(papof_handle* h, const SorPlanes& sp, const double* u, const double* v, double* u_out, double* v_out,
                    const double* im1, const double* im2, double* warp, double* phi_out, int H, int W, int planes,
                    bool do_warp = true, int row0 = 0, int row1 = -1, unsigned* wit = nullptr, int batch = 1,
                    const BatchK* bk = nullptr);
int update_flow(papof_handle* h, const SorPlanes& sp, double* u, double* v, int H, int W, const Rect& r);
int sor_prep(papof_handle* h, const double* phi, const double* imdxy, const double* imdx2, const double* imdy2,
             const double* rhs1, const double* rhs2, int H, int W, double alpha, double omega, const SorPlanes& out);
int sor_unpack(papof_handle* h, const SorPlanes& sp, double* du, double* dv, int H, int W);
Taps gaussian_taps(double sigma, int fsize);
Taps smooth5_taps();
Taps deriv5_taps();
Taps central3_taps();

struct SorBatch {
    int n;
    size_t coef, d, prog, tiny;
};
int sor_solve(papof_handle* h, const SorPlanes& sp, int H, int W, double alpha, double omega, int n_sor, int mode,
              const SorBatch* bt = nullptr);
int sor_blocked_depth(const papof_handle* h, int mode, int H, int W);
int sor_blocked_launch(papof_handle* h, const SorPlanes& sp, int H, int W, double alpha, double omega, int mode, int g,
                       int hs0, const Rect& out, const double* su, const double* sv, double* du, double* dv);
int sor_plan(const papof_handle* h, int H, int W, int n_sor, int mode, int* launches, int* depth);
int sor_check(papof_handle* h);
bool sor_strips_supported(const papof_handle* h, const SorPlanes& sp, int n_sor);
int sor_strips_begin(papof_handle* h, const SorPlanes& sp, int n_sor, int n_solves);
struct SorSplit {
    double* peer_du;
    unsigned* peer_prog;
    bool top_cut, bot_cut;
};
int sor_solve_bands(papof_handle* h, const SorPlanes& sp, int H, int W, double alpha, double omega, int n_sor,
                    unsigned* prog, int b0, int b1, const SorSplit* split = nullptr);
int sor_bind_plain(papof_handle* h, SorPlanes& sp, int H, int W, int n_sor);
constexpr size_t kTinyMaxCells = 8192;
bool sor_tiny_fits(const papof_handle* h, int H, int W, int n_sor);
bool sor_tiny_shape(int H, int W, int* cells_per_tile, int* waves);
int sor_alloc_tiny_planes(Arena& A, size_t cells, SorPlanes& sp);
size_t sor_counters_words(int H, int W, int n_sor);
int sor_counters_ensure(papof_handle* h, size_t words);
unsigned* sor_counters_clear(papof_handle* h, size_t offset_words, size_t words);
int sor_alloc_planes(Arena& A, int H, int W, int mode, int n_sor_cap, SorPlanes& sp);
int sor_bind(papof_handle* h, SorPlanes& sp, int H, int W, int n_sor);
int sor_group_size(const papof_handle* h, int H, int W, int n_sor);
int sor_reset_planes(papof_handle* h, const SorPlanes& sp);
int sor_reset_planes_batch(papof_handle* h, const SorPlanes& sp, int batch, size_t stride);
int sor_probe_dpp(papof_handle* h);

}
```

papteam_opticalflow_amd/csrc/flow_internal.h:

```cpp
#pragma once

#include <string>
#include <utility>
#include <vector>

#include "common.h"

namespace papof {

void set_last_error_text(const std::string& text);

constexpr int kTimerFused = PAPOF_N_TIMERS;
struct PhaseClock {
    papof_handle* h;
    bool on;
    std::vector<std::pair<int, std::pair<size_t, size_t>>> spans;
    size_t open = 0;
    int open_idx = -1;
    int err = PAPOF_OK;
    bool only_sor = false;
    bool stamps = false;
    std::vector<std::pair<int, int>> marks;
    std::vector<double> sor_span_sec;
    std::vector<int> sor_owner;
    size_t new_event() {
        if (h->events_used == h->events.size()) {
            hipEvent_t e;
            if (hipEventCreate(&e) != hipSuccess) {
                err = PAPOF_EDEVICE;
                return 0;
            }
            h->events.push_back(e);
        }
        hipEventRecord(h->events[h->events_used], h->stream);
        return h->events_used++;
    }
    void phase(int idx) {
        if (!on) return;
        if (stamps) {
            if (open_idx == PAPOF_T_PHASE5_SOR) {
                const size_t e = new_event();
                spans.push_back({PAPOF_T_PHASE5_SOR, {open, e}});
            }
            if (idx == PAPOF_T_PHASE5_SOR) {
                open = new_event();
                sor_owner.push_back(marks.empty() ? PAPOF_T_PHASE4_LINEARSYSTEM : marks.back().second);
            }
            const bool sor_edge = idx == PAPOF_T_PHASE5_SOR;
            open_idx = idx;
            if (only_sor || !h->stamps_dev || sor_edge) return;
            if (h->next_stamp && !marks.empty()) {
                marks.back().second = idx;
            } else if (h->stamps_used < h->stamps_cap) {
                const int slot = h->stamps_used++;
                h->next_stamp = h->stamps_dev + slot;
                marks.push_back({slot, idx});
            }
            return;
        }
        if (only_sor && idx != PAPOF_T_PHASE5_SOR && idx != PAPOF_T_TOTAL) {
            if (open_idx < 0) return;
            idx = -1;
        }
        const size_t e = new_event();
        if (open_idx >= 0) spans.push_back({open_idx, {open, e}});
        open = e;
        open_idx = idx;
    }
    void collect(double* t) {
        if (!on) return;
        for (auto& s : spans) {
            float ms = 0;
            if (hipEventElapsedTime(&ms, h->events[s.second.first], h->events[s.second.second]) == hipSuccess)
                t[s.first] += ms * 1e-3;
            if (s.first == PAPOF_T_PHASE5_SOR) sor_span_sec.push_back(ms * 1e-3);
        }
        for (size_t i = 0; i + 1 < marks.size(); i++) {
            const int idx = marks[i].second;
            if (marks[i + 1].first >= h->stamps_fetched) break;
            const unsigned long long a = h->stamps[marks[i].first], b = h->stamps[marks[i + 1].first];
            if (idx >= 0 && idx != PAPOF_T_PHASE5_SOR && b >= a) t[idx] += (double)(b - a) * 1e-8;
        }
        if (stamps && !marks.empty()) {
            for (size_t i = 0; i < sor_span_sec.size() && i < sor_owner.size(); i++)
                if (sor_owner[i] >= 0) t[sor_owner[i]] -= sor_span_sec[i];
            for (int own : {(int)PAPOF_T_PHASE4_LINEARSYSTEM, kTimerFused})
                if (t[own] < 0.0) t[own] = 0.0;
        }
    }
};

inline bool lap_proven(unsigned wit, unsigned epoch, bool nz_known, unsigned nz_a, unsigned nz_b) {
    const bool witness = wit == epoch || wit == (epoch ^ kLapNone);
    const bool all_zero = nz_known && nz_a != epoch && nz_b != epoch;
    return witness || all_zero;
}

struct Level {
    int w, h;
    double *p1, *p2;
};
struct PyrPlan {
    int sw, sh, src_level, fsize;
    double sigma, rate;
};

inline double effective_ratio(double ratio) { return ratio > 0.98 || ratio < 0.4 ? 0.75 : ratio; }
papof_params params_or_default(const papof_params* params);
struct CallPlan {
    double ratio = 0.75;
    int levels = 0, fc = 0;
    std::vector<Level> L;
    std::vector<PyrPlan> plan;
    std::vector<int> n_sor, n_outer;
    int n_sor_max = 0;
    long slots = 0;
    bool from_level0 = true;
    static int n_sor_at(const papof_params& P, int k) { return P.n_sor + k * P.n_sor_per_level; }
    static int n_outer_at(const papof_params& P, int k) { return P.n_outer + k * P.n_outer_per_level; }
    static long slots_for(const papof_params& P, int levels) {
        long s = 0;
        for (int k = 0; k < levels; k++) s += n_outer_at(P, k);
        return s;
    }
};
int call_plan(int H, int W, int C, int levels, const papof_params& P, CallPlan& cp);

inline unsigned* counters_base(const papof_handle* h) { return h->sync_words + 32; }
struct SolveCounters {
    struct PerLevel {
        size_t off = 0, per = 0;
    };
    std::vector<PerLevel> lv;
    size_t total = 0;
    SolveCounters() = default;
    template <class Words>
    SolveCounters(const CallPlan& cp, Words words, size_t solves_per_outer) : lv(cp.levels) {
        for (int k = 0; k < cp.levels; k++) {
            lv[k].per = words(k);
            lv[k].off = total;
            total += lv[k].per * (size_t)cp.n_outer[k] * solves_per_outer;
        }
    }
    unsigned* solve(const papof_handle* h, int k, size_t i) const { return counters_base(h) + lv[k].off + i * lv[k].per; }
};

int lap_next_epoch(papof_handle* h, hipStream_t stream);

inline int collect_total_and_sor(PhaseClock& total, PhaseClock& sorclk, double* timing) {
    if (total.err != PAPOF_OK || sorclk.err != PAPOF_OK) return PAPOF_EDEVICE;
    double tm[PAPOF_N_TIMERS + 1] = {};
    sorclk.collect(tm);
    total.collect(tm);
    for (int i = 0; timing && i < PAPOF_N_TIMERS; i++) timing[i] = tm[i];
    return PAPOF_OK;
}

struct StreamSwap {
    papof_handle* h;
    hipStream_t saved;
    StreamSwap(papof_handle* hh, hipStream_t s) : h(hh), saved(hh->stream) { h->stream = s; }
    ~StreamSwap() { h->stream = saved; }
};
int fork_prep(papof_handle* h, int levels, bool overlap);

size_t arena_bytes_for(int H, int W, int C, int levels, int n_sor_max, double ratio);
int ensure_arena(papof_handle* h, size_t bytes);
int check_params(const papof_params& P, int levels);
int pyramid_plan(int H, int W, double ratio, int nlev, std::vector<Level>& L, std::vector<PyrPlan>& plan);
int build_pyramid(papof_handle* h, const std::vector<Level>& L, const std::vector<PyrPlan>& plan, int C, bool second,
                  double* tmp_a, double* tmp_b);
int smooth_and_resize(papof_handle* h, const double* src, double* dst, double* tmp_a, double* tmp_b, const PyrPlan& p, int C,
                      int dh, int dw);
int feature_channels(int C);
int flow_batch_host(papof_handle* h, int n_pairs, int sequence, const void* const* frames, bool u8, int H, int W, int C, int levels,
                    const papof_params* params, double* const* vx, double* const* vy, double* const* warpI2, double* timing_sec);
int flow_device_planar(papof_handle* h, const double* f1, const double* f2, int H, int W, int C, int levels,
                       const papof_params& P, double* d_vx, double* d_vy, double* d_warp, double* timing,
                       const papof_tensor* init = nullptr);
int reduce_init(papof_handle* h, const papof_tensor* a, const papof_tensor* b, int pairs_a, int pairs_b, int H, int W,
                const std::vector<Level>& L, const std::vector<PyrPlan>& plan, double ratio, double* X, double* Y, double* T,
                size_t t_planes, double*& out);

}
```

papteam_opticalflow_amd/csrc/kernels.hip:

```cpp
#include "common.h"
#include "sampler.h"

#include <cmath>
#include <type_traits>

namespace papof {

namespace {

constexpr int BX = 64, BY = 4;

constexpr int tiles_of(int n, int t) { return (n + t - 1) / t; }
inline dim3 grid2d(int W, int H, int planes = 1) { return dim3(tiles_of(W, BX), tiles_of(H, BY), planes); }
inline Rect region(const Rect* rc, int W, int H) { return rc ? *rc : Rect{0, 0, W, H}; }
inline dim3 grid2d(const Rect& r, int planes = 1) { return grid2d(r.x1 - r.x0, r.y1 - r.y0, planes); }

__device__ __forceinline__ void stamp_now(unsigned long long* s) {
    if (s && (blockIdx.x | blockIdx.y | blockIdx.z | threadIdx.x | threadIdx.y) == 0u) *s = __builtin_amdgcn_s_memrealtime();
}
__global__ void k_stamp(unsigned long long* s) { stamp_now(s); }

__device__ __forceinline__ int clampi(int x, int n) {
    x = x < 0 ? 0 : x;
    return x > n - 1 ? n - 1 : x;
}

__device__ __forceinline__ bool xcd_tile(int ntx, int nty, int& tx, int& ty) {
    const int ntiles = ntx * nty, per = (ntiles + 7) >> 3;
    const int vt = (int)(blockIdx.x & 7u) * per + (int)(blockIdx.x >> 3);
    if ((int)(blockIdx.x >> 3) >= per || vt >= ntiles) return false;
    ty = vt / ntx;
    tx = vt - ty * ntx;
    return true;
}
static inline unsigned xcd_grid(int ntx, int nty) { return 8u * (unsigned)(((size_t)ntx * nty + 7) / 8); }

template <int HALF = -1, class At>
__device__ __forceinline__ double tap_sum(const Taps& f, At at, int half_rt = HALF) {
    const int half = HALF >= 0 ? HALF : half_rt;
    double acc = 0.0;
#pragma unroll
    for (int l = -half; l <= half; l++) acc += at(l) * f.t[l + half];
    return acc;
}

__device__ __forceinline__ void blend_imdt(double s1, double s2, double& blend, double& imdt) {
    double t = s1;
    t *= 0.4;
    t += s2 * 0.6;
    blend = t;
    imdt = s2 - s1;
}

__device__ __forceinline__ double phi_value(double uc, double vc, double ur, double vr, double ud, double vd, bool right,
                                            bool down) {
    const double ux = right ? ur - uc : 0.0;
    const double uy = down ? ud - uc : 0.0;
    const double vx = right ? vr - vc : 0.0;
    const double vy = down ? vd - vc : 0.0;
    const double t = ux * ux + uy * uy + vx * vx + vy * vy;
    return 0.5 / sqrt(t + 0.001 * 0.001);
}
__device__ __forceinline__ double phi_at(const double* __restrict__ u, const double* __restrict__ v, int i, int j, int H,
                                         int W) {
    const size_t o = (size_t)i * W + j;
    const double uc = u[o], vc = v[o];
    double ur = 0.0, vr = 0.0, ud = 0.0, vd = 0.0;
    if (j < W - 1) {
        ur = u[o + 1];
        vr = v[o + 1];
    }
    if (i < H - 1) {
        ud = u[o + W];
        vd = v[o + W];
    }
    return phi_value(uc, vc, ur, vr, ud, vd, j < W - 1, i < H - 1);
}

__device__ __forceinline__ bool leaves_image(double x, double y, int W, int H) {
    return x < 0 || x > W - 1 || y < 0 || y > H - 1;
}
__device__ __forceinline__ double bilinear_inside(double g0, double g1, double g2, double g3, double dx, double dy) {
    const double ex = 1.0 - dx, ey = 1.0 - dy;
    double res = 0.0;
    res += g0 * (ex * ey);
    res += g1 * (ex * dy);
    res += g2 * (dx * ey);
    res += g3 * (dx * dy);
    return res;
}
__device__ __forceinline__ double bilinear_inside_at(const double* __restrict__ p, int W, int H, double x, double y) {
    const int x0 = (int)x, y0 = (int)y;
    const int x1 = min(x0 + 1, W - 1), y1 = min(y0 + 1, H - 1);
    return bilinear_inside(p[y0 * W + x0], p[y1 * W + x0], p[y0 * W + x1], p[y1 * W + x1], x - x0, y - y0);
}

__device__ __forceinline__ bool lap_valid(double d) { return d > 0 && d < 1000000; }
__device__ __forceinline__ bool lap_witness(double d, double thr, bool sampled = true) {
    return sampled && d >= thr && d < 1000000;
}
__device__ __forceinline__ bool lap_one_in_sixteen(int tbx, int tby) { return ((tbx + 5 * tby) & 15) == 0; }
__device__ __forceinline__ bool lap_samples_here(int nblocks, int tbx, int tby) {
    return nblocks <= 256 || lap_one_in_sixteen(tbx, tby);
}

__global__ void k_hwc_to_planar(const double* __restrict__ hwc, double* __restrict__ planar, int H, int W, int C) {
    const int j = blockIdx.x * BX + threadIdx.x, i = blockIdx.y * BY + threadIdx.y;
    if (j >= W || i >= H) return;
    const size_t o = (size_t)i * W + j, np = (size_t)H * W;
    hwc += blockIdx.z * np * C;
    planar += blockIdx.z * np * C;
    for (int k = 0; k < C; k++) planar[k * np + o] = hwc[o * C + k];
}

__global__ void k_hwc_u8_to_planar(const unsigned char* __restrict__ hwc, double* __restrict__ planar, int H, int W,
                                   int C) {
    const int j = blockIdx.x * BX + threadIdx.x, i = blockIdx.y * BY + threadIdx.y;
    if (j >= W || i >= H) return;
    const size_t o = (size_t)i * W + j, np = (size_t)H * W;
    hwc += blockIdx.z * np * C;
    planar += blockIdx.z * np * C;
    for (int k = 0; k < C; k++) planar[k * np + o] = (double)hwc[o * C + k] / 255.0;
}

__global__ void k_planar_to_hwc(const double* __restrict__ planar, double* __restrict__ hwc, int H, int W, int C) {
    const int j = blockIdx.x * BX + threadIdx.x, i = blockIdx.y * BY + threadIdx.y;
    if (j >= W || i >= H) return;
    const size_t o = (size_t)i * W + j, np = (size_t)H * W;
    for (int k = 0; k < C; k++) hwc[o * C + k] = planar[k * np + o];
}

__device__ __forceinline__ double tensor_load(const void* p, int dtype, long long o) {
    if (dtype == PAPOF_DTYPE_U8) return (double)static_cast<const unsigned char*>(p)[o] / 255.0;
    if (dtype == PAPOF_DTYPE_F32) return (double)static_cast<const float*>(p)[o];
    return static_cast<const double*>(p)[o];
}

__global__ __launch_bounds__(256) void k_ingest_frames(const papof_tensor a, const papof_tensor b, int pairs,
                                                       double* __restrict__ planar, long long H, long long W, long long C,
                                                       long long total) {
    const long long i = (long long)blockIdx.x * blockDim.x + threadIdx.x;
    if (i >= total) return;
    const long long np = H * W, f = i / (np * C), r = i - f * np * C, c = r / np, px = r - c * np, row = px / W,
                    col = px - row * W;
    const bool second = pairs && (f & 1);
    const long long fi = pairs ? f >> 1 : f;
    const long long o = fi * (second ? b.stride[0] : a.stride[0]) + row * (second ? b.stride[1] : a.stride[1]) +
                        col * (second ? b.stride[2] : a.stride[2]) + c * (second ? b.stride[3] : a.stride[3]);
    planar[i] = tensor_load(second ? b.data : a.data, second ? b.dtype : a.dtype, o);
}

constexpr double kInitMax = 1e6;
__device__ __forceinline__ bool init_refused(double x) { return !(fabs(x) <= kInitMax); }

__global__ __launch_bounds__(256) void k_init_check(const papof_tensor t, long long H, long long W, long long total,
                                                    unsigned* __restrict__ flag) {
    const long long i = (long long)blockIdx.x * blockDim.x + threadIdx.x;
    if (i >= total) return;
    const long long np = H * W, p = i / (np * 2), r = i - p * np * 2, c = r / np, px = r - c * np, row = px / W,
                    col = px - row * W;
    const long long o = p * t.stride[0] + row * t.stride[1] + col * t.stride[2] + c * t.stride[3];
    if (init_refused(tensor_load(t.data, t.dtype, o))) atomicOr(flag, 1u);
}

__global__ __launch_bounds__(256) void k_init_sanitize(double* __restrict__ planar, long long total) {
    const long long i = (long long)blockIdx.x * blockDim.x + threadIdx.x;
    if (i >= total) return;
    if (init_refused(planar[i])) planar[i] = 0.0;
}

__global__ __launch_bounds__(256) void k_emit_outputs(const double* __restrict__ src, const papof_tensor dst, int comp_major,
                                                      long long H, long long W, long long K, long long total) {
    const long long i = (long long)blockIdx.x * blockDim.x + threadIdx.x;
    if (i >= total) return;
    const long long np = H * W, p = i / (np * K), r = i - p * np * K;
    const long long k = comp_major ? r / np : r % K, px = comp_major ? r - k * np : r / K, row = px / W, col = px - row * W;
    const long long o = p * dst.stride[0] + row * dst.stride[1] + col * dst.stride[2] + k * dst.stride[3];
    const double v = src[i];
    if (dst.dtype == PAPOF_DTYPE_F32)
        static_cast<float*>(dst.data)[o] = (float)v;
    else
        static_cast<double*>(dst.data)[o] = v;
}

constexpr int kFbTX = 64, kFbTY = 4;
__global__ __launch_bounds__(kFbTX * kFbTY) void k_fb_check(const papof_tensor fw, const papof_tensor bw, const papof_tensor mask,
                                                         int H, int W, double a1, double a2) {
    const int tx = (W + kFbTX - 1) / kFbTX;
    const int x = (int)(blockIdx.x % tx) * kFbTX + threadIdx.x, r = (int)(blockIdx.x / tx) * kFbTY + threadIdx.y;
    if (x >= W || r >= H) return;
    const long long p = blockIdx.y >> 1;
    const int dir = blockIdx.y & 1;
    const papof_tensor& f = dir ? bw : fw;
    const papof_tensor& b = dir ? fw : bw;
    const long long of = p * f.stride[0] + r * f.stride[1] + x * f.stride[2];
    const double u = load_flow(f, of), v = load_flow(f, of + f.stride[3]);
    const double X = (double)x + u, Y = (double)r + v;
    bool occluded = true;
    if (X >= 0 && X <= (double)(W - 1) && Y >= 0 && Y <= (double)(H - 1)) {
        double bu, bv;
        sample_flow(b, p * b.stride[0], taps_at(X, Y, H, W), bu, bv);
        occluded = !fb_passes(u, v, bu, bv, a1, a2);
    }
    static_cast<unsigned char*>(mask.data)[p * mask.stride[0] + r * mask.stride[1] + x * mask.stride[2] + dir * mask.stride[3]] =
        occluded ? 1 : 0;
}

__global__ void k_filter_h(const double* __restrict__ src, double* __restrict__ dst, int H, int W, Taps f, Rect rc) {
    const int j = rc.x0 + blockIdx.x * BX + threadIdx.x, i = rc.y0 + blockIdx.y * BY + threadIdx.y;
    if (j >= rc.x1 || i >= rc.y1) return;
    const size_t np = (size_t)H * W;
    const double* row = src + blockIdx.z * np + (size_t)i * W;
    dst[blockIdx.z * np + (size_t)i * W + j] = tap_sum(f, [&](int l) { return row[clampi(j + l, W)]; }, f.fsize);
}

__global__ void k_filter_v(const double* __restrict__ src, double* __restrict__ dst, int H, int W, Taps f, Rect rc) {
    const int j = rc.x0 + blockIdx.x * BX + threadIdx.x, i = rc.y0 + blockIdx.y * BY + threadIdx.y;
    if (j >= rc.x1 || i >= rc.y1) return;
    const size_t np = (size_t)H * W;
    const double* p = src + blockIdx.z * np + j;
    dst[blockIdx.z * np + (size_t)i * W + j] = tap_sum(f, [&](int l) { return p[(size_t)clampi(i + l, H) * W]; }, f.fsize);
}

#ifndef PAPOF_V_HVROWS
#define PAPOF_V_HVROWS 64
#endif
constexpr int kHvRows = PAPOF_V_HVROWS, kHvMaxF = 4;
template <int F>
__global__ __launch_bounds__(256) void k_filter_hv(const double* __restrict__ src, double* __restrict__ dst, int H, int W,
                                                   Taps fh, Taps fv) {
    __shared__ double hs[kHvRows + 2 * kHvMaxF][BX];
    const int j = blockIdx.x * BX + threadIdx.x, i0 = blockIdx.y * kHvRows;
    const int f = F >= 0 ? F : fv.fsize, fx = F >= 0 ? F : fh.fsize;
    const size_t np = (size_t)H * W;
    const double* plane = src + blockIdx.z * np;
    if (j < W) {
        for (int r = threadIdx.y; r < kHvRows + 2 * f; r += BY) {
            const double* row = plane + (size_t)clampi(i0 + r - f, H) * W;
            hs[r][threadIdx.x] = tap_sum<F>(fh, [&](int l) { return row[clampi(j + l, W)]; }, fx);
        }
    }
    __syncthreads();
    if (j >= W) return;
    for (int r = threadIdx.y; r < kHvRows; r += BY) {
        const int i = i0 + r;
        if (i >= H) break;
        dst[blockIdx.z * np + (size_t)i * W + j] = tap_sum<F>(fv, [&](int l) { return hs[r + l + f][threadIdx.x]; }, f);
    }
}

#ifndef PAPOF_V_HVSTAGED
#define PAPOF_V_HVSTAGED 1
#endif
#ifndef PAPOF_V_HVSROWS
#define PAPOF_V_HVSROWS 16
#endif
constexpr int kHvsRows = PAPOF_V_HVSROWS;
template <int F>
__global__ __launch_bounds__(256) void k_filter_hv_staged(const double* __restrict__ src, double* __restrict__ dst, int H,
                                                          int W, Taps fh, Taps fv) {
    __shared__ double raw[kHvsRows + 2 * F][BX + 2 * F];
    __shared__ double hs[kHvsRows + 2 * F][BX];
    int tx, ty;
    if (!xcd_tile((W + BX - 1) / BX, (H + kHvsRows - 1) / kHvsRows, tx, ty)) return;
    const int j0 = tx * BX, i0 = ty * kHvsRows;
    const size_t np = (size_t)H * W;
    const double* plane = src + blockIdx.z * np;
    constexpr int kCells = (kHvsRows + 2 * F) * (BX + 2 * F);
    for (int c = threadIdx.y * BX + threadIdx.x; c < kCells; c += BX * BY) {
        const int r = c / (BX + 2 * F), cc = c - r * (BX + 2 * F);
        raw[r][cc] = plane[(size_t)clampi(i0 + r - F, H) * W + clampi(j0 + cc - F, W)];
    }
    __syncthreads();
    for (int r = threadIdx.y; r < kHvsRows + 2 * F; r += BY) {
        hs[r][threadIdx.x] = tap_sum<F>(fh, [&](int l) { return raw[r][threadIdx.x + F + l]; });
    }
    __syncthreads();
    const int j = j0 + threadIdx.x;
    if (j >= W) return;
    for (int r = threadIdx.y; r < kHvsRows; r += BY) {
        const int i = i0 + r;
        if (i >= H) break;
        dst[blockIdx.z * np + (size_t)i * W + j] = tap_sum<F>(fv, [&](int l) { return hs[r + l + F][threadIdx.x]; });
    }
}

struct BilinearTaps {
    int o[4];
    double s[4];
};

__device__ __forceinline__ BilinearTaps bilinear_taps(int W, int H, double x, double y) {
    BilinearTaps b;
    const int xx = (int)x, yy = (int)y;
    double dx = x - xx, dy = y - yy;
    dx = dx > 1 ? 1.0 : dx;
    dx = dx < 0 ? 0.0 : dx;
    dy = dy > 1 ? 1.0 : dy;
    dy = dy < 0 ? 0.0 : dy;
#pragma unroll
    for (int m = 0; m <= 1; m++)
#pragma unroll
        for (int n = 0; n <= 1; n++) {
            const int u = clampi(xx + m, W), v = clampi(yy + n, H);
            b.o[m * 2 + n] = v * W + u;
            b.s[m * 2 + n] = fabs((double)(1 - m) - dx) * fabs((double)(1 - n) - dy);
        }
    return b;
}

__device__ __forceinline__ double bilinear_apply(const double* __restrict__ p, const BilinearTaps& b) {
    double acc = 0.0;
#pragma unroll
    for (int t = 0; t < 4; t++) acc += p[b.o[t]] * b.s[t];
    return acc;
}

__global__ void k_resize(const double* __restrict__ src, double* __restrict__ dst, int sh, int sw, int dh, int dw,
                         double xr, double yr, int use_post, double post, Rect rc, unsigned long long* stamp) {
    stamp_now(stamp);
    int tbx, tby;
    if (!xcd_tile((rc.x1 - rc.x0 + BX - 1) / BX, (rc.y1 - rc.y0 + BY - 1) / BY, tbx, tby)) return;
    const int j = rc.x0 + tbx * BX + threadIdx.x, i = rc.y0 + tby * BY + threadIdx.y;
    if (j >= rc.x1 || i >= rc.y1) return;
    const double x = (double)(j + 1) / xr - 1;
    const double y = (double)(i + 1) / yr - 1;
    const BilinearTaps b = bilinear_taps(sw, sh, x, y);
    double r = bilinear_apply(src + blockIdx.z * (size_t)sh * sw, b);
    if (use_post) r *= post;
    dst[blockIdx.z * (size_t)dh * dw + (size_t)i * dw + j] = r;
}

template <int C>
__device__ __forceinline__ double gray_at(const double* __restrict__ im, size_t np, size_t o) {
    if (C == 3) return im[o] * .299 + im[np + o] * .587 + im[2 * np + o] * .114;
    return im[o];
}

template <int C>
__global__ void k_im2feature(const double* __restrict__ im, double* __restrict__ feat, int H, int W, Taps d) {
    const int j = blockIdx.x * BX + threadIdx.x, i = blockIdx.y * BY + threadIdx.y;
    if (j >= W || i >= H) return;
    const size_t np = (size_t)H * W, o = (size_t)i * W + j;
    double gx = 0.0, gy = 0.0;
#pragma unroll
    for (int l = -2; l <= 2; l++) gx += gray_at<C>(im, np, (size_t)i * W + clampi(j + l, W)) * d.t[l + 2];
#pragma unroll
    for (int l = -2; l <= 2; l++) gy += gray_at<C>(im, np, (size_t)clampi(i + l, H) * W + j) * d.t[l + 2];
    feat[o] = gray_at<C>(im, np, o);
    feat[np + o] = gx;
    feat[2 * np + o] = gy;
    if (C == 3) {
        feat[3 * np + o] = im[np + o] - im[o];
        feat[4 * np + o] = im[np + o] - im[2 * np + o];
    }
}

#ifndef PAPOF_V_FEATROWS
#define PAPOF_V_FEATROWS 16
#endif
constexpr int kFeatRows = PAPOF_V_FEATROWS;
template <int C, bool BATCH = false>
__global__ __launch_bounds__(256) void k_im2feature_tiled(const double* __restrict__ im, double* __restrict__ feat, int H,
                                                          int W, Taps d, unsigned* __restrict__ nz, unsigned mark,
                                                          size_t b_im, size_t b_feat, size_t b_nz) {
    __shared__ double g[kFeatRows + 4][BX + 4];
    int tx, ty;
    if (!xcd_tile((W + BX - 1) / BX, (H + kFeatRows - 1) / kFeatRows, tx, ty)) return;
    const int j0 = tx * BX, i0 = ty * kFeatRows;
    const size_t np = (size_t)H * W;
    if (BATCH) {
        im += blockIdx.y * b_im;
        feat += blockIdx.y * b_feat;
        if (nz != nullptr) nz += blockIdx.y * b_nz;
    }
    for (int c = threadIdx.y * BX + threadIdx.x; c < (kFeatRows + 4) * (BX + 4); c += BX * BY) {
        const int r = c / (BX + 4), cc = c - r * (BX + 4);
        g[r][cc] = gray_at<C>(im, np, (size_t)clampi(i0 + r - 2, H) * W + clampi(j0 + cc - 2, W));
    }
    __syncthreads();
    const int j = j0 + threadIdx.x;
    bool any[5] = {false, false, false, false, false};
    if (j < W) {
        for (int r = threadIdx.y; r < kFeatRows; r += BY) {
            const int i = i0 + r;
            if (i >= H) break;
            const size_t o = (size_t)i * W + j;
            double gx = 0.0, gy = 0.0;
#pragma unroll
            for (int l = -2; l <= 2; l++) gx += g[r + 2][threadIdx.x + 2 + l] * d.t[l + 2];
#pragma unroll
            for (int l = -2; l <= 2; l++) gy += g[r + 2 + l][threadIdx.x + 2] * d.t[l + 2];
            const double f0 = g[r + 2][threadIdx.x + 2];
            feat[o] = f0;
            feat[np + o] = gx;
            feat[2 * np + o] = gy;
            any[0] |= f0 != 0.0;
            any[1] |= gx != 0.0;
            any[2] |= gy != 0.0;
            if (C == 3) {
                const double gg = im[np + o];
                const double f3 = gg - im[o], f4 = gg - im[2 * np + o];
                feat[3 * np + o] = f3;
                feat[4 * np + o] = f4;
                any[3] |= f3 != 0.0;
                any[4] |= f4 != 0.0;
            }
        }
    }
    if (nz != nullptr) {
#pragma unroll
        for (int k = 0; k < (C == 3 ? 5 : 3); k++)
            if (__ballot(any[k]) != 0ull && threadIdx.x == 0) nz[k] = mark;
    }
}

__global__ void k_central3_all(const double* __restrict__ src, double* __restrict__ gx, double* __restrict__ gy,
                               double* __restrict__ gxy, int H, int W, Taps c3) {
    int tbx, tby;
    if (!xcd_tile((W + BX - 1) / BX, (H + BY - 1) / BY, tbx, tby)) return;
    const int j = tbx * BX + threadIdx.x, i = tby * BY + threadIdx.y;
    if (j >= W || i >= H) return;
    const size_t np = (size_t)H * W;
    const double* p = src + blockIdx.z * np;
    const auto hrow = [&](int ii) {
        const double* row = p + (size_t)ii * W;
        double acc = 0.0;
#pragma unroll
        for (int l = -1; l <= 1; l++) acc += row[clampi(j + l, W)] * c3.t[l + 1];
        return acc;
    };
    const double hx[3] = {hrow(clampi(i - 1, H)), hrow(i), hrow(clampi(i + 1, H))};
    double vy = 0.0, vxy = 0.0;
#pragma unroll
    for (int l = -1; l <= 1; l++) vy += p[(size_t)clampi(i + l, H) * W + j] * c3.t[l + 1];
#pragma unroll
    for (int l = -1; l <= 1; l++) vxy += hx[l + 1] * c3.t[l + 1];
    const size_t o = blockIdx.z * np + (size_t)i * W + j;
    gx[o] = hx[1];
    gy[o] = vy;
    gxy[o] = vxy;
}

__device__ __forceinline__ void warp_pixel(const double* __restrict__ im1, const double* __restrict__ im2,
                                           double* __restrict__ out, double fx, double fy, int i, int j, int H,
                                           int W, int planes) {
    const size_t np = (size_t)H * W, o = (size_t)i * W + j;
    const double y = i + fy;
    const double x = j + fx;
    if (leaves_image(x, y, W, H)) {
        for (int k = 0; k < planes; k++) out[k * np + o] = im1[k * np + o];
        return;
    }
    for (int k = 0; k < planes; k++) out[k * np + o] = bilinear_inside_at(im2 + k * np, W, H, x, y);
}

__global__ void k_warp(const double* __restrict__ im1, const double* __restrict__ im2, const double* __restrict__ vx,
                       const double* __restrict__ vy, double* __restrict__ out, int H, int W, int planes, Rect rc,
                       unsigned long long* stamp) {
    stamp_now(stamp);
    const int j = rc.x0 + blockIdx.x * BX + threadIdx.x, i = rc.y0 + blockIdx.y * BY + threadIdx.y;
    if (j >= rc.x1 || i >= rc.y1) return;
    const size_t o = (size_t)i * W + j;
    warp_pixel(im1, im2, out, vx[o], vy[o], i, j, H, W, planes);
}

__global__ void k_smooth_v_blend(const double* __restrict__ tmp, const double* __restrict__ im1s,
                                 double* __restrict__ blend, double* __restrict__ imdt, int H, int W, Taps g, Rect rc) {
    const int j = rc.x0 + blockIdx.x * BX + threadIdx.x, i = rc.y0 + blockIdx.y * BY + threadIdx.y;
    if (j >= rc.x1 || i >= rc.y1) return;
    const size_t np = (size_t)H * W, o = blockIdx.z * np + (size_t)i * W + j;
    const double* p = tmp + blockIdx.z * np + j;
    const double s2 = tap_sum<2>(g, [&](int l) { return p[(size_t)clampi(i + l, H) * W]; });
    blend_imdt(im1s[o], s2, blend[o], imdt[o]);
}

constexpr int kFuseRows = 16;
__global__ __launch_bounds__(256) void k_smooth_hv_blend(const double* __restrict__ warp,
                                                         const double* __restrict__ im1s,
                                                         double* __restrict__ blend, double* __restrict__ imdt, int H,
                                                         int W, Taps g, unsigned long long* stamp, int row0, int row1) {
    __shared__ double hs[kFuseRows + 4][BX];
    stamp_now(stamp);
    const int j = blockIdx.x * BX + threadIdx.x, i0 = row0 + blockIdx.y * kFuseRows;
    const size_t np = (size_t)H * W;
    const double* src = warp + blockIdx.z * np;
    if (j < W) {
        for (int r = threadIdx.y; r < kFuseRows + 4; r += BY) {
            const double* row = src + (size_t)clampi(i0 + r - 2, H) * W;
            hs[r][threadIdx.x] = tap_sum<2>(g, [&](int l) { return row[clampi(j + l, W)]; });
        }
    }
    __syncthreads();
    if (j >= W) return;
    for (int r = threadIdx.y; r < kFuseRows; r += BY) {
        const int i = i0 + r;
        if (i >= row1) break;
        const size_t o = blockIdx.z * np + (size_t)i * W + j;
        const double s2 = tap_sum<2>(g, [&](int l) { return hs[r + l + 2][threadIdx.x]; });
        blend_imdt(im1s[o], s2, blend[o], imdt[o]);
    }
}

__device__ __forceinline__ double warp_value(const double* __restrict__ im1, const double* __restrict__ im2, double fx,
                                             double fy, int i, int j, int H, int W) {
    const double y = i + fy;
    const double x = j + fx;
    if (leaves_image(x, y, W, H)) return im1[(size_t)i * W + j];
    return bilinear_inside_at(im2, W, H, x, y);
}
#ifndef PAPOF_V_WSROWS
#define PAPOF_V_WSROWS 16
#endif
#ifndef PAPOF_V_WSBATCH
#define PAPOF_V_WSBATCH 3
#endif
constexpr int kWsBatch = PAPOF_V_WSBATCH;
constexpr int kWsRows = PAPOF_V_WSROWS;
__global__ __launch_bounds__(256) void k_warp_smooth_blend(const double* __restrict__ im1, const double* __restrict__ im2,
                                                           const double* __restrict__ u, const double* __restrict__ v,
                                                           const double* __restrict__ im1s, double* __restrict__ blend,
                                                           double* __restrict__ imdt, int H, int W, Taps g,
                                                           unsigned long long* stamp, unsigned* __restrict__ wit,
                                                           double wit_thr, unsigned mark, double* __restrict__ phi_out) {
    __shared__ double raw[kWsRows + 4][BX + 4];
    __shared__ double hs[kWsRows + 4][BX];
    stamp_now(stamp);
    const int j0 = blockIdx.x * BX, i0 = blockIdx.y * kWsRows;
    const size_t np = (size_t)H * W;
    const double *p1 = im1 + blockIdx.z * np, *p2 = im2 + blockIdx.z * np;
    const bool exhaustive = wit != nullptr && gridDim.x == 1u && gridDim.y == 1u;
    bool ex_hit = false, ex_valid = false;
    const bool sampler = wit != nullptr && !exhaustive && threadIdx.y == 0u &&
                         lap_samples_here((int)(gridDim.x * gridDim.y), (int)blockIdx.x, (int)blockIdx.y);
    constexpr int kWitStride = (kWsRows + 4) * (BX + 4) / 64;
    const int wr = (int)(threadIdx.x * kWitStride) / (BX + 4), wc = (int)(threadIdx.x * kWitStride) - wr * (BX + 4);
    double own1 = 0.0;
    if (sampler) own1 = p1[(size_t)clampi(i0 + wr - 2, H) * W + clampi(j0 + wc - 2, W)];
    constexpr int kCells = (kWsRows + 4) * (BX + 4), kPer = (kCells + BX * BY - 1) / (BX * BY);
    const int tid = threadIdx.y * BX + threadIdx.x;
#pragma unroll
    for (int q0 = 0; q0 < kPer; q0 += kWsBatch) {
        double fx[kWsBatch], fy[kWsBatch], val[kWsBatch][4];
        int off[kWsBatch];
#pragma unroll
        for (int q = 0; q < kWsBatch; q++) {
            const int c = min(tid + (q0 + q) * BX * BY, kCells - 1);
            const int r = c / (BX + 4), cc = c - r * (BX + 4);
            const int i = clampi(i0 + r - 2, H), j = clampi(j0 + cc - 2, W);
            off[q] = i * W + j;
            fx[q] = u[off[q]];
            fy[q] = v[off[q]];
        }
        bool outside[kWsBatch];
#pragma unroll
        for (int q = 0; q < kWsBatch; q++) {
            const int c = min(tid + (q0 + q) * BX * BY, kCells - 1);
            const int r = c / (BX + 4), cc = c - r * (BX + 4);
            const int i = clampi(i0 + r - 2, H), j = clampi(j0 + cc - 2, W);
            double y = i + fy[q], x = j + fx[q];
            outside[q] = leaves_image(x, y, W, H);
            if (outside[q]) {
                x = j;
                y = i;
            }
            const int x0 = (int)x, y0 = (int)y;
            const int x1 = min(x0 + 1, W - 1), y1 = min(y0 + 1, H - 1);
            val[q][0] = p2[y0 * W + x0];
            val[q][1] = p2[y1 * W + x0];
            val[q][2] = p2[y0 * W + x1];
            val[q][3] = p2[y1 * W + x1];
            fx[q] = x - x0;
            fy[q] = y - y0;
        }
#pragma unroll
        for (int q = 0; q < kWsBatch; q++) {
            const int c = tid + (q0 + q) * BX * BY;
            if (c >= kCells) continue;
            const int r = c / (BX + 4), cc = c - r * (BX + 4);
            const double res =
                outside[q] ? p1[off[q]] : bilinear_inside(val[q][0], val[q][1], val[q][2], val[q][3], fx[q], fy[q]);
            raw[r][cc] = res;
            if (exhaustive) {
                const double d = fabs(p1[off[q]] - res);
                ex_valid = ex_valid || lap_valid(d);
                ex_hit = ex_hit || lap_witness(d, wit_thr);
            }
        }
    }
    __syncthreads();
    if (exhaustive) {
        const int any_hit = __syncthreads_or(ex_hit ? 1 : 0), any_valid = __syncthreads_or(ex_valid ? 1 : 0);
        if (tid == 0 && (any_hit || !any_valid)) wit[blockIdx.z] = any_hit ? mark : (mark ^ kLapNone);
    }
// ... 616 lines not shown
        const PhiAround p{ph[orow + 1][ocol + 1], n.left ? ph[orow + 1][ocol] : 0.0, n.up ? ph[orow][ocol + 1] : 0.0};
        const SystemCell c = system_cell<true>(s, p, cross_at<true>(u, o, W, n), cross_at<true>(v, o, W, n), n, alpha, omega);
        if (SKEW) {
            stage_cell(stage, orow, ocol, c);
        } else {
            out.q[0][o] = c.phi;
            out.q[1][o] = c.xy;
            out.q[2][o] = c.a1;
            out.q[3][o] = c.a2;
            out.q[4][o] = c.b1;
            out.q[5][o] = c.b2;
        }
    }
    if (!SKEW) return;
    __syncthreads();
    store_skew_tile(stage, tid, ib, j0, row1, W, sk, reinterpret_cast<double2s*>(out.q[0]),
                    reinterpret_cast<double2s*>(out.q[2]), reinterpret_cast<double2s*>(out.q[4]));
}

template <bool SKEW>
__global__ void k_sor_prep(const double* __restrict__ phi, const double* __restrict__ imdxy,
                           const double* __restrict__ imdx2, const double* __restrict__ imdy2,
                           const double* __restrict__ rhs1, const double* __restrict__ rhs2, int H, int W,
                           double alpha, double omega, SkewIdx sk, double* __restrict__ o_phi,
                           double* __restrict__ o_xy, double* __restrict__ o_a1, double* __restrict__ o_a2,
                           double* __restrict__ o_b1, double* __restrict__ o_b2) {
    const int j = blockIdx.x * BX + threadIdx.x, i = blockIdx.y * BY + threadIdx.y;
    if (j >= W || i >= H) return;
    const size_t o = (size_t)i * W + j;
    double a1, a2;
    const Nbrs n = nbrs_at(i, j, H, W);
    sor_diagonals<true>(phi_around<true>(phi, o, W, n), n, imdx2[o], imdy2[o], alpha, omega, a1, a2);
    const size_t q = sor_index<SKEW>(i, j, W, sk);
    o_phi[q] = phi[o];
    o_xy[q] = imdxy[o];
    o_a1[q] = a1;
    o_a2[q] = a2;
    o_b1[q] = rhs1[o];
    o_b2[q] = rhs2[o];
}

template <bool SKEW>
__global__ void k_sor_unpack(const double* __restrict__ sdu, const double* __restrict__ sdv,
                             double* __restrict__ du, double* __restrict__ dv, int H, int W, SkewIdx sk) {
    const int j = blockIdx.x * BX + threadIdx.x, i = blockIdx.y * BY + threadIdx.y;
    if (j >= W || i >= H) return;
    const size_t o = (size_t)i * W + j;
    if (SKEW) {
        const size_t q = 2 * dudv_cell(i, j, sk);
        du[o] = sdu[q];
        dv[o] = sdu[q + 1];
    } else {
        du[o] = sdu[o];
        dv[o] = sdv[o];
    }
}

__global__ void k_update_warp(const double* __restrict__ sdu, const double* __restrict__ sdv, double* __restrict__ u,
                              double* __restrict__ v, const double* __restrict__ im1,
                              const double* __restrict__ im2, double* __restrict__ warp, int H, int W, int planes, Rect rc,
                              int do_warp, unsigned long long* stamp) {
    stamp_now(stamp);
    const int j = rc.x0 + blockIdx.x * BX + threadIdx.x, i = rc.y0 + blockIdx.y * BY + threadIdx.y;
    if (j >= rc.x1 || i >= rc.y1) return;
    const size_t o = (size_t)i * W + j;
    double fu = u[o], fv = v[o];
    fu += sdu[o];
    fv += sdv[o];
    u[o] = fu;
    v[o] = fv;
    if (do_warp) warp_pixel(im1, im2, warp, fu, fv, i, j, H, W, planes);
}

template <bool SKEW, bool BATCH = false>
__global__ void k_update_warp_phi(const double* __restrict__ sdu, const double* __restrict__ sdv, SkewIdx sk,
                                  const double* __restrict__ u, const double* __restrict__ v,
                                  double* __restrict__ u_out, double* __restrict__ v_out,
                                  const double* __restrict__ im1, const double* __restrict__ im2,
                                  double* __restrict__ warp, double* __restrict__ phi_out, int H, int W, int planes,
                                  int do_warp, unsigned long long* stamp, int row0, int row1, unsigned* __restrict__ wit,
                                  double wit_thr, unsigned mark, BatchK bk) {
    stamp_now(stamp);
    if (BATCH) {
        const size_t p = blockIdx.y;
        sdu += p * bk.d;
        sdv += p * bk.d;
        u += p * bk.uv;
        v += p * bk.uv;
        u_out += p * bk.uv;
        v_out += p * bk.uv;
        batch_frames(bk, p, im1, im2);
        if (wit != nullptr) wit += p * bk.wit;
    }
    int tbx, tby;
    if (!xcd_tile((W + BX - 1) / BX, (row1 - row0 + BY - 1) / BY, tbx, tby)) return;
    const int j = tbx * BX + threadIdx.x, i = row0 + tby * BY + threadIdx.y;
    if (j >= W || i >= row1) return;
    const size_t o = (size_t)i * W + j;
    const auto inc = [&](int ii, int jj, double& a, double& b) {
        if (SKEW) {
            const double2s c = reinterpret_cast<const double2s*>(sdu)[dudv_cell(ii, jj, sk)];
            a = c.x;
            b = c.y;
        } else {
            a = sdu[(size_t)ii * W + jj];
            b = sdv[(size_t)ii * W + jj];
        }
    };
    double a, b;
    inc(i, j, a, b);
    double fu = u[o], fv = v[o];
    fu += a;
    fv += b;
    u_out[o] = fu;
    v_out[o] = fv;
    if (wit != nullptr) {
        const int bw = min(W - tbx * BX, BX), bh = min(row1 - (row0 + tby * BY), BY);
        const int lin = threadIdx.y * bw + threadIdx.x;
        const size_t np = (size_t)H * W;
        if (np <= 65536) {
            for (int k = bw * bh >= planes ? lin % planes : lin; k < planes; k += bw * bh) {
                const double w = warp_value(im1 + k * np, im2 + k * np, fu, fv, i, j, H, W);
                const double d = fabs(im1[k * np + o] - w);
                if (lap_witness(d, wit_thr)) wit[k] = mark;
            }
        } else if (lap_one_in_sixteen(tbx, tby))
        for (int k = lin; k < planes; k += bw * bh) {
            const double w = warp_value(im1 + k * np, im2 + k * np, fu, fv, i, j, H, W);
            const double d = fabs(im1[k * np + o] - w);
            if (lap_witness(d, wit_thr)) wit[k] = mark;
        }
    }
    if (phi_out != nullptr) {
        double ur = 0.0, vr = 0.0, ud = 0.0, vd = 0.0;
        if (j < W - 1) {
            inc(i, j + 1, a, b);
            ur = u[o + 1];
            vr = v[o + 1];
            ur += a;
            vr += b;
        }
        if (i < H - 1) {
            inc(i + 1, j, a, b);
            ud = u[o + W];
            vd = v[o + W];
            ud += a;
            vd += b;
        }
        phi_out[o] = phi_value(fu, fv, ur, vr, ud, vd, j < W - 1, i < H - 1);
    }
    if (do_warp) warp_pixel(im1, im2, warp, fu, fv, i, j, H, W, planes);
}

template <bool BATCH>
__global__ void k_bicubic(const double* __restrict__ im1, const double* __restrict__ im2,
                          const double* __restrict__ gx, const double* __restrict__ gy,
                          const double* __restrict__ gxy, const double* __restrict__ vx,
                          const double* __restrict__ vy, double* __restrict__ out, int H, int W, int C, Rect rc,
                          unsigned long long* stamp, int planar_out, int clamp, BatchK bk) {
    if (BATCH) {
        const size_t p = blockIdx.y;
        const ptrdiff_t o1 = (ptrdiff_t)batch_frames(bk, p, im1, im2);
        const ptrdiff_t o2 = bk.bw != 0 && p >= bk.bw ? o1 - 2 * (ptrdiff_t)bk.fr : o1;
        gx += o2;
        gy += o2;
        gxy += o2;
        vx += p * bk.uv;
        vy += p * bk.uv;
        out += p * bk.out;
    }
    stamp_now(stamp);
    int tbx, tby;
    if (!xcd_tile((rc.x1 - rc.x0 + BX - 1) / BX, (rc.y1 - rc.y0 + BY - 1) / BY, tbx, tby)) return;
    const int j = rc.x0 + tbx * BX + threadIdx.x, i = rc.y0 + tby * BY + threadIdx.y;
    if (j >= rc.x1 || i >= rc.y1) return;
    const size_t np = (size_t)H * W, o = (size_t)i * W + j;
    const size_t ostride = planar_out ? np : 1, obase = planar_out ? o : o * C;
    const double x = j + vx[o];
    const double y = i + vy[o];
    if (x < 0 || x > W - 1 || y < 0 || y > H - 1) {
        for (int k = 0; k < C; k++) {
            double r = im1[k * np + o];
            if (clamp) {
                r = r < 0 ? 0.0 : r;
                r = r > 1 ? 1.0 : r;
            }
            out[obase + k * ostride] = r;
        }
        return;
    }
    int x0 = (int)x, y0 = (int)y;
    int x1 = x0 + 1, y1 = y0 + 1;
    x0 = clampi(x0, W);
    x1 = clampi(x1, W);
    y0 = clampi(y0, H);
    y1 = clampi(y1, H);
    const double dx = x - x0, dy = y - y0;
    const double dx2 = dx * dx, dy2 = dy * dy;
    const double dx3 = dx * dx2, dy3 = dy * dy2;
    const size_t a = (size_t)y0 * W + x0, b = (size_t)y0 * W + x1, c = (size_t)y1 * W + x0, d = (size_t)y1 * W + x1;
    for (int k = 0; k < C; k++) {
        const double *f = im2 + k * np, *px = gx + k * np, *py = gy + k * np, *pz = gxy + k * np;
        const double fA = f[a], fB = f[b], fC = f[c], fD = f[d];
        const double xA = px[a], xB = px[b], xC = px[c], xD = px[d];
        const double yA = py[a], yB = py[b], yC = py[c], yD = py[d];
        const double zA = pz[a], zB = pz[b], zC = pz[c], zD = pz[d];
        const double c00 = fA;
        const double c10 = xA;
        const double c20 = -3 * fA + 3 * fB - 2 * xA - xB;
        const double c30 = 2 * fA - 2 * fB + xA + xB;
        const double c01 = yA;
        const double c11 = zA;
        const double c21 = -3 * yA + 3 * yB - 2 * zA - zB;
        const double c31 = 2 * yA - 2 * yB + zA + zB;
        const double c02 = -3 * fA + 3 * fC - 2 * yA - yC;
        const double c12 = -3 * xA + 3 * xC - 2 * zA - zC;
        const double c22 = 9 * fA - 9 * fB - 9 * fC + 9 * fD + 6 * xA + 3 * xB - 6 * xC - 3 * xD + 6 * yA - 6 * yB +
                           3 * yC - 3 * yD + 4 * zA + 2 * zB + 2 * zC + zD;
        const double c32 = -6 * fA + 6 * fB + 6 * fC - 6 * fD - 3 * xA - 3 * xB + 3 * xC + 3 * xD - 4 * yA + 4 * yB -
                           2 * yC + 2 * yD - 2 * zA - 2 * zB - zC - zD;
        const double c03 = 2 * fA - 2 * fC + yA + yC;
        const double c13 = 2 * xA - 2 * xC + zA + zC;
        const double c23 = -6 * fA + 6 * fB + 6 * fC - 6 * fD - 4 * xA - 2 * xB + 4 * xC + 2 * xD - 3 * yA + 3 * yB -
                           3 * yC + 3 * yD - 2 * zA - zB - 2 * zC - zD;
        const double c33 = 4 * fA - 4 * fB - 4 * fC + 4 * fD + 2 * xA + 2 * xB - 2 * xC - 2 * xD + 2 * yA - 2 * yB +
                           2 * yC - 2 * yD + zA + zB + zC + zD;
        double r = c00 + c01 * dy + c02 * dy2 + c03 * dy3 + c10 * dx + c11 * dx * dy + c12 * dx * dy2 +
                   c13 * dx * dy3 + c20 * dx2 + c21 * dx2 * dy + c22 * dx2 * dy2 + c23 * dx2 * dy3 + c30 * dx3 +
                   c31 * dx3 * dy + c32 * dx3 * dy2 + c33 * dx3 * dy3;
        if (clamp) {
            r = r < 0 ? 0.0 : r;
            r = r > 1 ? 1.0 : r;
        }
        out[obase + k * ostride] = r;
    }
}

__global__ void k_flow_quantize16(const double* __restrict__ vx, const double* __restrict__ vy,
                                  unsigned short* __restrict__ q, size_t n) {
    const size_t i = (size_t)blockIdx.x * blockDim.x + threadIdx.x;
    if (i >= n) return;
    double a = vx[i], b = vy[i];
    a = (a < -200) ? -200.0 : a;
    a = (a > 200) ? 200.0 : a;
    b = (b < -200) ? -200.0 : b;
    b = (b > 200) ? 200.0 : b;
    q[i * 2] = (unsigned short)((a + 200) * 160);
    q[i * 2 + 1] = (unsigned short)((b + 200) * 160);
}

__global__ void k_flow_dequantize16(const unsigned short* __restrict__ q, double* __restrict__ vx,
                                    double* __restrict__ vy, size_t n) {
    const size_t i = (size_t)blockIdx.x * blockDim.x + threadIdx.x;
    if (i >= n) return;
    vx[i] = (double)q[i * 2] / 160 - 200;
    vy[i] = (double)q[i * 2 + 1] / 160 - 200;
}

__global__ void k_flow_mag_minmax(const double* __restrict__ vx, const double* __restrict__ vy, size_t n,
                                  double* __restrict__ partial) {
    __shared__ double smin[256], smax[256];
    double lo = INFINITY, hi = -INFINITY;
    for (size_t i = (size_t)blockIdx.x * blockDim.x + threadIdx.x; i < n; i += (size_t)gridDim.x * blockDim.x) {
        const double m = sqrt(vx[i] * vx[i] + vy[i] * vy[i]);
        lo = m < lo ? m : lo;
        hi = m > hi ? m : hi;
    }
    smin[threadIdx.x] = lo;
    smax[threadIdx.x] = hi;
    __syncthreads();
    for (int s = 128; s > 0; s >>= 1) {
        if ((int)threadIdx.x < s) {
            smin[threadIdx.x] = fmin(smin[threadIdx.x], smin[threadIdx.x + s]);
            smax[threadIdx.x] = fmax(smax[threadIdx.x], smax[threadIdx.x + s]);
        }
        __syncthreads();
    }
    if (threadIdx.x == 0) {
        partial[2 * blockIdx.x] = smin[0];
        partial[2 * blockIdx.x + 1] = smax[0];
    }
}

__global__ void k_flow_bgr(const double* __restrict__ vx, const double* __restrict__ vy, size_t n,
                           const double* __restrict__ partial, int nblocks, unsigned char* __restrict__ bgr) {
    const size_t i = (size_t)blockIdx.x * blockDim.x + threadIdx.x;
    if (i >= n) return;
    double lo = INFINITY, hi = -INFINITY;
    for (int b = 0; b < nblocks; b++) {
        lo = fmin(lo, partial[2 * b]);
        hi = fmax(hi, partial[2 * b + 1]);
    }
    const double x = vx[i], y = vy[i];
    const double mag = sqrt(x * x + y * y);
    double ang = atan2(y, x);
    if (ang < 0) ang += 2 * M_PI;
    const unsigned char H = (unsigned char)(int)(ang * 180 / M_PI / 2);
    const double scale = hi > lo ? 255.0 / (hi - lo) : 0.0;
    const unsigned char V = (unsigned char)(int)((mag - lo) * scale);
    const float v = V * (1.f / 255.f);
    float h = H * (6.f / 180.f);
    int sector = (int)floorf(h);
    h -= sector;
    sector = ((sector % 6) + 6) % 6;
    const float tab[4] = {v, 0.f, v * (1.f - h), v * h};
    const int sd[6][3] = {{1, 3, 0}, {1, 0, 2}, {3, 0, 1}, {0, 2, 1}, {0, 1, 3}, {2, 1, 0}};
    bgr[i * 3] = (unsigned char)(int)rintf(tab[sd[sector][0]] * 255.f);
    bgr[i * 3 + 1] = (unsigned char)(int)rintf(tab[sd[sector][1]] * 255.f);
    bgr[i * 3 + 2] = (unsigned char)(int)rintf(tab[sd[sector][2]] * 255.f);
}

}

Taps gaussian_taps(double sigma, int fsize) {
    Taps f{};
    f.fsize = fsize;
    double sum = 0;
    const double s2 = sigma * sigma * 2;
    for (int i = -fsize; i <= fsize; i++) {
        f.t[i + fsize] = std::exp(-(double)(i * i) / s2);
        sum += f.t[i + fsize];
    }
    for (int i = 0; i < 2 * fsize + 1; i++) f.t[i] /= sum;
    return f;
}

Taps smooth5_taps() {
    Taps f{};
    f.fsize = 2;
    const double g[5] = {0.02, 0.11, 0.74, 0.11, 0.02};
    for (int i = 0; i < 5; i++) f.t[i] = g[i];
    return f;
}

Taps deriv5_taps() {
    Taps f{};
    f.fsize = 2;
    const double d[5] = {1, -8, 0, 8, -1};
    for (int i = 0; i < 5; i++) {
        f.t[i] = d[i];
        f.t[i] /= 12;
    }
    return f;
}

Taps central3_taps() {
    Taps f{};
    f.fsize = 1;
    f.t[0] = -0.5;
    f.t[1] = 0;
    f.t[2] = 0.5;
    return f;
}

#define LAUNCH_CHECK() PAPOF_HIP(hipGetLastError())

const SkewIdx kNoSkew{};
const BatchK kNoBatch{};

static bool rows_of(int row0, int& row1, int H, int& rc) {
    if (row1 < 0) row1 = H;
    rc = row0 < 0 || row1 > H ? PAPOF_EINVAL : PAPOF_OK;
    return rc == PAPOF_OK && row1 > row0;
}

static double lap_wit_threshold(int H, int W) { return 2e-20 * (double)H * (double)W; }

template <class F>
static auto with_flags(F f) {
    return f();
}
template <class F, class... Rest>
static auto with_flags(F f, bool flag, Rest... rest) {
    return flag ? with_flags([&](auto... t) { return f(std::true_type{}, t...); }, rest...)
                : with_flags([&](auto... t) { return f(std::false_type{}, t...); }, rest...);
}

int hwc_to_planar(papof_handle* h, const double* hwc, double* planar, int H, int W, int C, int frames) {
    hipLaunchKernelGGL(k_hwc_to_planar, grid2d(W, H, frames), dim3(BX, BY), 0, h->stream, hwc, planar, H, W, C);
    LAUNCH_CHECK();
    return PAPOF_OK;
}

int hwc_u8_to_planar(papof_handle* h, const unsigned char* hwc, double* planar, int H, int W, int C, int frames) {
    hipLaunchKernelGGL(k_hwc_u8_to_planar, grid2d(W, H, frames), dim3(BX, BY), 0, h->stream, hwc, planar, H, W, C);
    LAUNCH_CHECK();
    return PAPOF_OK;
}

int ingest_frames(papof_handle* h, const papof_tensor& a, const papof_tensor* b, double* planar, int H, int W, int C,
                  int frames) {
    const long long total = (long long)frames * H * W * C, blocks = (total + 255) / 256;
    if (total <= 0) return PAPOF_OK;
    if (blocks > 0x7fffffffLL) return PAPOF_EINVAL;
    hipLaunchKernelGGL(k_ingest_frames, dim3((unsigned)blocks), dim3(256), 0, h->stream, a, b ? *b : a, b ? 1 : 0, planar,
                       (long long)H, (long long)W, (long long)C, total);
    LAUNCH_CHECK();
    return PAPOF_OK;
}

int init_check(papof_handle* h, const papof_tensor& t, int pairs, int H, int W, unsigned* flag) {
    const long long total = (long long)pairs * H * W * 2, blocks = (total + 255) / 256;
    if (total <= 0) return PAPOF_OK;
    if (blocks > 0x7fffffffLL) return PAPOF_EINVAL;
    hipLaunchKernelGGL(k_init_check, dim3((unsigned)blocks), dim3(256), 0, h->stream, t, (long long)H, (long long)W, total,
                       flag);
    LAUNCH_CHECK();
    return PAPOF_OK;
}

int init_sanitize(papof_handle* h, double* planar, size_t n) {
    const long long total = (long long)n, blocks = (total + 255) / 256;
    if (total <= 0) return PAPOF_OK;
    if (blocks > 0x7fffffffLL) return PAPOF_EINVAL;
    hipLaunchKernelGGL(k_init_sanitize, dim3((unsigned)blocks), dim3(256), 0, h->stream, planar, total);
    LAUNCH_CHECK();
    return PAPOF_OK;
}

bool filter_hv_needs_tmp(const Taps& fh, const Taps& fv) { return fh.fsize > kHvMaxF || fv.fsize > kHvMaxF; }

int emit_outputs(papof_handle* h, const double* src, const papof_tensor& dst, bool comp_major, int H, int W, int K, int pairs) {
    const long long total = (long long)pairs * H * W * K, blocks = (total + 255) / 256;
    if (total <= 0) return PAPOF_OK;
    if (blocks > 0x7fffffffLL) return PAPOF_EINVAL;
    hipLaunchKernelGGL(k_emit_outputs, dim3((unsigned)blocks), dim3(256), 0, h->stream, src, dst, comp_major ? 1 : 0,
                       (long long)H, (long long)W, (long long)K, total);
    LAUNCH_CHECK();
    return PAPOF_OK;
}

int fb_check(papof_handle* h, hipStream_t st, const papof_tensor& fw, const papof_tensor& bw, const papof_tensor& mask,
             int pairs, int H, int W, double a1, double a2) {
    const long long tiles = (long long)tiles_of(W, kFbTX) * tiles_of(H, kFbTY);
    if (pairs <= 0 || tiles <= 0) return PAPOF_OK;
    if (tiles > kMaxTiles) return PAPOF_EINVAL;
    const auto at = [](const papof_tensor& t, long long items) {
        papof_tensor r = t;
        r.data = static_cast<char*>(t.data) + items * t.stride[0] * dtype_bytes(t.dtype);
        return r;
    };
    for (int p0 = 0; p0 < pairs; p0 += 32767) {
        const int n = std::min(32767, pairs - p0);
        hipLaunchKernelGGL(k_fb_check, dim3((unsigned)tiles, 2 * n), dim3(kFbTX, kFbTY), 0, st, at(fw, p0), at(bw, p0),
                           at(mask, p0), H, W, a1, a2);
        LAUNCH_CHECK();
    }
    return PAPOF_OK;
}

int planar_to_hwc(papof_handle* h, const double* planar, double* hwc, int H, int W, int C) {
    hipLaunchKernelGGL(k_planar_to_hwc, grid2d(W, H), dim3(BX, BY), 0, h->stream, planar, hwc, H, W, C);
    LAUNCH_CHECK();
    return PAPOF_OK;
}

int filter_h(papof_handle* h, const double* src, double* dst, int H, int W, int planes, const Taps& f, const Rect* rc) {
    const Rect r = region(rc, W, H);
    if (r.empty()) return PAPOF_OK;
    hipLaunchKernelGGL(k_filter_h, grid2d(r, planes), dim3(BX, BY), 0, h->stream, src, dst, H, W, f, r);
    LAUNCH_CHECK();
    return PAPOF_OK;
}

int filter_v(papof_handle* h, const double* src, double* dst, int H, int W, int planes, const Taps& f, const Rect* rc) {
    const Rect r = region(rc, W, H);
    if (r.empty()) return PAPOF_OK;
    hipLaunchKernelGGL(k_filter_v, grid2d(r, planes), dim3(BX, BY), 0, h->stream, src, dst, H, W, f, r);
    LAUNCH_CHECK();
    return PAPOF_OK;
}

int central3_planes(papof_handle* h, const double* src, double* gx, double* gy, double* gxy, int H, int W, int planes) {
    hipLaunchKernelGGL(k_central3_all, dim3(xcd_grid(tiles_of(W, BX), tiles_of(H, BY)), 1, planes), dim3(BX, BY), 0, h->stream, src, gx, gy, gxy, H, W,
                       central3_taps());
    LAUNCH_CHECK();
    return PAPOF_OK;
}

int filter_hv(papof_handle* h, const double* src, double* dst, double* tmp, int H, int W, int planes, const Taps& fh,
              const Taps& fv) {
    if (fh.fsize > kHvMaxF || fv.fsize > kHvMaxF) {
        if (!tmp) return PAPOF_EINVAL;
        PAPOF_TRY(filter_h(h, src, tmp, H, W, planes, fh));
        return filter_v(h, tmp, dst, H, W, planes, fv);
    }
    const dim3 grid(tiles_of(W, BX), tiles_of(H, kHvRows), planes), block(BX, BY);
    const int f = fh.fsize == fv.fsize ? fh.fsize : -1;
    if (PAPOF_V_HVSTAGED && f >= 1 && f <= 3) {
        const dim3 sgrid(xcd_grid(tiles_of(W, BX), tiles_of(H, kHvsRows)), 1, planes);
        if (f == 1)
            hipLaunchKernelGGL(k_filter_hv_staged<1>, sgrid, block, 0, h->stream, src, dst, H, W, fh, fv);
        else if (f == 2)
            hipLaunchKernelGGL(k_filter_hv_staged<2>, sgrid, block, 0, h->stream, src, dst, H, W, fh, fv);
        else
            hipLaunchKernelGGL(k_filter_hv_staged<3>, sgrid, block, 0, h->stream, src, dst, H, W, fh, fv);
        LAUNCH_CHECK();
        return PAPOF_OK;
    }
    if (f == 1)
        hipLaunchKernelGGL(k_filter_hv<1>, grid, block, 0, h->stream, src, dst, H, W, fh, fv);
    else if (f == 2)
        hipLaunchKernelGGL(k_filter_hv<2>, grid, block, 0, h->stream, src, dst, H, W, fh, fv);
    else if (f == 3)
        hipLaunchKernelGGL(k_filter_hv<3>, grid, block, 0, h->stream, src, dst, H, W, fh, fv);
    else
        hipLaunchKernelGGL(k_filter_hv<-1>, grid, block, 0, h->stream, src, dst, H, W, fh, fv);
    LAUNCH_CHECK();
    return PAPOF_OK;
}

int resize(papof_handle* h, const double* src, double* dst, int sh, int sw, int planes, int dh, int dw, double xr,
           double yr, bool use_post, double post, const Rect* rc) {
    const Rect r = region(rc, dw, dh);
    if (r.empty()) return PAPOF_OK;
    hipLaunchKernelGGL(k_resize, dim3(xcd_grid(tiles_of(r.x1 - r.x0, BX), tiles_of(r.y1 - r.y0, BY)), 1, planes), dim3(BX, BY), 0, h->stream, src, dst, sh, sw, dh, dw, xr, yr,
                       use_post ? 1 : 0, post, r, take_stamp(h));
    LAUNCH_CHECK();
    return PAPOF_OK;
}

int im2feature(papof_handle* h, const double* im, double* feat, int H, int W, int C, unsigned* nz, int frames, size_t nz_stride) {
    const size_t np = (size_t)H * W;
    if (C == 3) {
        hipLaunchKernelGGL((frames > 1 ? k_im2feature_tiled<3, true> : k_im2feature_tiled<3, false>), dim3(xcd_grid(tiles_of(W, BX), tiles_of(H, kFeatRows)), frames), dim3(BX, BY), 0,
                           h->stream, im, feat, H, W, deriv5_taps(), nz, h->lap_epoch, 3 * np, 5 * np, nz_stride);
    } else if (C == 1) {
        hipLaunchKernelGGL((frames > 1 ? k_im2feature_tiled<1, true> : k_im2feature_tiled<1, false>), dim3(xcd_grid(tiles_of(W, BX), tiles_of(H, kFeatRows)), frames), dim3(BX, BY), 0,
                           h->stream, im, feat, H, W, deriv5_taps(), nz, h->lap_epoch, np, 3 * np, nz_stride);
    } else {
        if (frames != 1) return PAPOF_EINVAL;
        PAPOF_HIP(hipMemcpyAsync(feat, im, sizeof(double) * (size_t)H * W * C, hipMemcpyDeviceToDevice, h->stream));
        return PAPOF_OK;
    }
    LAUNCH_CHECK();
    return PAPOF_OK;
}

int warp_bilinear(papof_handle* h, const double* im1, const double* im2, const double* vx, const double* vy,
                  double* out, int H, int W, int planes, const Rect* rc) {
    const Rect r = region(rc, W, H);
    if (r.empty()) return PAPOF_OK;
    hipLaunchKernelGGL(k_warp, grid2d(r), dim3(BX, BY), 0, h->stream, im1, im2, vx, vy, out, H, W, planes, r,
                       take_stamp(h));
    LAUNCH_CHECK();
    return PAPOF_OK;
}

int smooth_v_blend(papof_handle* h, const double* tmp, const double* im1s, double* blend, double* imdt, int H,
                   int W, int planes, const Rect* rc) {
    const Rect r = region(rc, W, H);
    if (r.empty()) return PAPOF_OK;
    hipLaunchKernelGGL(k_smooth_v_blend, grid2d(r, planes), dim3(BX, BY), 0, h->stream, tmp, im1s, blend, imdt, H, W,
                       smooth5_taps(), r);
    LAUNCH_CHECK();
    return PAPOF_OK;
}

static SkewIdx skew_idx(const SorPlanes& sp) {
    return SkewIdx{sp.sd.hp, sp.sd.qt, sp.sd.rt, sp.sd.nb, sp.sd.npos_d, sp.sd.dpar, sp.sd.band_rows, sp.sd.koff, sp.sd.poff};
}

static Increment increment_of(const SorPlanes* prev, const double* gm = nullptr, const double* lap = nullptr) {
    if (!prev) return Increment{nullptr, nullptr, 0, kNoSkew, gm, lap};
    return Increment{prev->du, prev->dv, prev->skew ? 1 : 0, prev->skew ? skew_idx(*prev) : kNoSkew,
                     gm, lap};
}

int smooth_hv_blend(papof_handle* h, const double* warp, const double* im1s, double* blend, double* imdt, int H,
                    int W, int planes, int row0, int row1) {
    int rc;
    if (!rows_of(row0, row1, H, rc)) return rc;
    hipLaunchKernelGGL(k_smooth_hv_blend, dim3(tiles_of(W, BX), tiles_of(row1 - row0, kFuseRows), planes),
                       dim3(BX, BY), 0, h->stream, warp, im1s, blend, imdt, H, W, smooth5_taps(), take_stamp(h), row0,
                       row1);
    LAUNCH_CHECK();
    return PAPOF_OK;
}

int warp_smooth_blend(papof_handle* h, const double* im1, const double* im2, const double* u, const double* v,
                      const double* im1s, double* blend, double* imdt, int H, int W, int planes, unsigned* wit,
                      double* phi_out) {
    hipLaunchKernelGGL(k_warp_smooth_blend, dim3(tiles_of(W, BX), tiles_of(H, kWsRows), planes), dim3(BX, BY), 0,
                       h->stream, im1, im2, u, v, im1s, blend, imdt, H, W, smooth5_taps(), take_stamp(h), wit,
                       lap_wit_threshold(H, W), h->lap_epoch, phi_out);
    LAUNCH_CHECK();
    return PAPOF_OK;
}

int compute_phi(papof_handle* h, const double* u, const double* v, const SorPlanes* prev, double* phi, int H, int W,
                const Rect* rc) {
    const Rect r = region(rc, W, H);
    if (r.empty()) return PAPOF_OK;
    hipLaunchKernelGGL(k_phi, grid2d(r), dim3(BX, BY), 0, h->stream, u, v, increment_of(prev), phi, H, W, r,
                       take_stamp(h));
    LAUNCH_CHECK();
    return PAPOF_OK;
}

int assemble_system(papof_handle* h, const double* blend, const double* imdt, const double* phi, const double* u,
                    const double* v, int H, int W, int planes, double alpha, double omega, const SorPlanes& out,
                    double* opt_imdx2, double* opt_imdy2, const SorPlanes* prev, const Rect* rc, const double* gm,
                    const double* lap) {
    const Increment I = increment_of(prev, gm, lap);
    const Rect r = region(rc, W, H);
    if (r.empty()) return PAPOF_OK;
    if (out.skew) {
        if (rc && (r.x0 != 0 || r.x1 != W)) return PAPOF_EINVAL;
        const bool fast = I.du == nullptr && I.gm == nullptr && I.lap == nullptr;
        const auto kern = planes == 5   ? (fast ? k_assemble_skew<5, true> : k_assemble_skew<5, false>)
                          : planes == 3 ? (fast ? k_assemble_skew<3, true> : k_assemble_skew<3, false>)
                                        : k_assemble_skew<0, false>;
        hipLaunchKernelGGL(kern, dim3(tiles_of(W, kTileJ), tiles_of(r.y1 - r.y0, kAsmRows)),
                           dim3(256), 0, h->stream, blend, imdt, phi, u, v, H, W, planes, alpha, omega, skew_idx(out),
                           (double2s*)out.phi, (double2s*)out.a1, (double2s*)out.b1, opt_imdx2, opt_imdy2,
                           deriv5_taps(), I, take_stamp(h), r.y0, r.y1);
    } else {
        hipLaunchKernelGGL(k_assemble, grid2d(r), dim3(BX, BY), 0, h->stream, blend, imdt, phi, u, v, H, W, planes,
                           alpha, omega, out.phi, out.xy, out.a1, out.a2, out.b1, out.b2, opt_imdx2, opt_imdy2,
                           deriv5_taps(), I, r, take_stamp(h));
    }
    LAUNCH_CHECK();
    return PAPOF_OK;
}

int flow_system(papof_handle* h, const double* im1, const double* im2, const double* u, const double* v, const double* im1s,
                int H, int W, int planes, double alpha, double omega, const SorPlanes& out, unsigned* wit, int row0, int row1,
                int batch, const BatchK* bk) {
    if (planes != 5 && planes != 3) return PAPOF_EINVAL;
    if ((unsigned long long)H * (unsigned long long)W > (1ull << 29)) return PAPOF_EINVAL;
    int rc;
    if (!rows_of(row0, row1, H, rc)) return rc;
    const dim3 grid(xcd_grid(tiles_of(W, kFT), tiles_of(row1 - row0, kFT)), batch);
    const SixPlanes six{{out.phi, out.xy, out.a1, out.a2, out.b1, out.b2}};
    const auto kern = with_flags([](auto five, auto skew, auto batched, auto one_column) {
        return &k_flow_system<five.value ? 5 : 3, skew.value, batched.value, one_column.value>;
    }, planes == 5, out.skew, batch > 1, W == 1);
    hipLaunchKernelGGL(kern, grid, dim3(kFT * kFT), 0, h->stream, im1, im2, u, v, im1s, H, W, alpha, omega,
                       out.skew ? skew_idx(out) : kNoSkew, six, smooth5_taps(), deriv5_taps(),
                       take_stamp(h), wit, lap_wit_threshold(H, W), h->lap_epoch, row0, row1, bk ? *bk : kNoBatch);
    LAUNCH_CHECK();
    return PAPOF_OK;
}

int laplacian(papof_handle* h, const double* in, const double* weight, double* out, int H, int W) {
    hipLaunchKernelGGL(k_laplacian, grid2d(W, H), dim3(BX, BY), 0, h->stream, in, weight, out, H, W);
    LAUNCH_CHECK();
    return PAPOF_OK;
}

int update_warp_phi(papof_handle* h, const SorPlanes& sp, const double* u, const double* v, double* u_out, double* v_out,
                    const double* im1, const double* im2, double* warp, double* phi_out, int H, int W, int planes,
                    bool do_warp, int row0, int row1, unsigned* wit, int batch, const BatchK* bk) {
    if (batch > 1 && (warp || phi_out || do_warp)) return PAPOF_EINVAL;
    if (u == u_out || v == v_out) return PAPOF_EINVAL;
    int rc;
    if (!rows_of(row0, row1, H, rc)) return rc;
    const dim3 grid(xcd_grid(tiles_of(W, BX), tiles_of(row1 - row0, BY)), batch);
    const auto kern = with_flags([](auto skew, auto batched) { return &k_update_warp_phi<skew.value, batched.value>; },
                                 sp.skew, batch > 1);
    hipLaunchKernelGGL(kern, grid, dim3(BX, BY), 0, h->stream, sp.du, sp.dv, sp.skew ? skew_idx(sp) : kNoSkew, u, v, u_out,
                       v_out, im1, im2, warp, phi_out, H, W, planes, do_warp ? 1 : 0, take_stamp(h), row0, row1, wit,
                       lap_wit_threshold(H, W), h->lap_epoch, bk ? *bk : kNoBatch);
    LAUNCH_CHECK();
    return PAPOF_OK;
}

int update_flow(papof_handle* h, const SorPlanes& sp, double* u, double* v, int H, int W, const Rect& r) {
    if (sp.skew) return PAPOF_EINVAL;
    if (r.empty()) return PAPOF_OK;
    hipLaunchKernelGGL(k_update_warp, grid2d(r), dim3(BX, BY), 0, h->stream, sp.du, sp.dv, u, v, nullptr, nullptr, nullptr,
                       H, W, 0, r, 0, take_stamp(h));
    LAUNCH_CHECK();
    return PAPOF_OK;
}

int flow_quantize16(papof_handle* h, const double* vx, const double* vy, unsigned short* q, size_t n) {
    if (!n) return PAPOF_OK;
    hipLaunchKernelGGL(k_flow_quantize16, dim3((unsigned)((n + 255) / 256)), dim3(256), 0, h->stream, vx, vy, q, n);
    LAUNCH_CHECK();
    return PAPOF_OK;
}

int flow_dequantize16(papof_handle* h, const unsigned short* q, double* vx, double* vy, size_t n) {
    if (!n) return PAPOF_OK;
    hipLaunchKernelGGL(k_flow_dequantize16, dim3((unsigned)((n + 255) / 256)), dim3(256), 0, h->stream, q, vx, vy, n);
    LAUNCH_CHECK();
    return PAPOF_OK;
}

int flow_to_bgr(papof_handle* h, const double* vx, const double* vy, size_t n, double* partial ,
                unsigned char* bgr) {
    if (!n) return PAPOF_OK;
    const int nblocks = 256;
    hipLaunchKernelGGL(k_flow_mag_minmax, dim3(nblocks), dim3(256), 0, h->stream, vx, vy, n, partial);
    hipLaunchKernelGGL(k_flow_bgr, dim3((unsigned)((n + 255) / 256)), dim3(256), 0, h->stream, vx, vy, n, partial,
                       nblocks, bgr);
    LAUNCH_CHECK();
    return PAPOF_OK;
}

int bicubic_warp(papof_handle* h, const double* im1, const double* im2, const double* gx, const double* gy,
                 const double* gxy, const double* vx, const double* vy, double* out_hwc, int H, int W, int C,
                 const Rect* rc, bool planar_out, bool clamp, int batch, const BatchK* bk) {
    const Rect r = region(rc, W, H);
    if (r.empty()) return PAPOF_OK;
    hipLaunchKernelGGL(batch > 1 ? k_bicubic<true> : k_bicubic<false>, dim3(xcd_grid(tiles_of(r.x1 - r.x0, BX), tiles_of(r.y1 - r.y0, BY)), batch), dim3(BX, BY), 0, h->stream, im1, im2, gx, gy, gxy, vx, vy, out_hwc, H, W,
                       C, r, take_stamp(h), planar_out ? 1 : 0, clamp ? 1 : 0, bk ? *bk : kNoBatch);
    LAUNCH_CHECK();
    return PAPOF_OK;
}

constexpr int kGmBlocks = 256, kGmThreads = 256, kGmMaxC = 8;
static __global__ __launch_bounds__(kGmThreads) void k_gm_partial(const double* __restrict__ im1,
                                                           const double* __restrict__ im2, size_t np, int C,
                                                           const double* __restrict__ gm, double* __restrict__ partial) {
    __shared__ double red[kGmThreads];
    double acc[kGmMaxC][4];
    for (int k = 0; k < kGmMaxC; k++) acc[k][0] = acc[k][1] = acc[k][2] = acc[k][3] = 0.0;
    for (size_t o = (size_t)blockIdx.x * kGmThreads + threadIdx.x; o < np; o += (size_t)kGmBlocks * kGmThreads) {
#pragma unroll
        for (int k = 0; k < kGmMaxC; k++) {
            if (k >= C) break;
            double t = im1[k * np + o] - im2[k * np + o];
            t *= t;
            const double alpha_k = gm[k], sigma = gm[C + k], beta = gm[2 * C + k], s2 = gm[3 * C + k], b2 = gm[4 * C + k];
            double w1 = exp(-t / (2 * s2)) / (2 * 3.1415927 * sigma) * alpha_k;
            double w2 = exp(-t / (2 * b2)) / (2 * 3.1415927 * beta) * (1 - alpha_k);
            const double s = w1 + w2;
            w1 /= s;
            w2 /= s;
            acc[k][0] += w1;
            acc[k][1] += w2;
            acc[k][2] += w1 * t;
            acc[k][3] += w2 * t;
        }
    }
    for (int k = 0; k < C; k++)
        for (int q = 0; q < 4; q++) {
            red[threadIdx.x] = acc[k][q];
            __syncthreads();
            for (int s = kGmThreads / 2; s > 0; s >>= 1) {
                if ((int)threadIdx.x < s) red[threadIdx.x] += red[threadIdx.x + s];
                __syncthreads();
            }
            if (threadIdx.x == 0) partial[((size_t)blockIdx.x * kGmMaxC + k) * 4 + q] = red[0];
            __syncthreads();
        }
}

static __global__ void k_gm_mstep(const double* __restrict__ partial, int C, double prior, double* __restrict__ gm) {
    const int k = threadIdx.x;
    if (k >= C) return;
    double t1 = 0.0, t2 = 0.0, s1 = 0.05, s2 = 0.5;
    for (int b = 0; b < kGmBlocks; b++) {
        const double* p = partial + ((size_t)b * kGmMaxC + k) * 4;
        t1 += p[0];
        t2 += p[1];
        s1 += p[2];
        s2 += p[3];
    }
    const double alpha = t1 / (t1 + t2) * (1 - prior) + 0.95 * prior;
    const double sigma = sqrt(s1 / t1);
    const double beta = sqrt(s2 / t2) * (1 - prior) + 0.3 * prior;
    gm[k] = alpha;
    gm[C + k] = sigma;
    gm[2 * C + k] = beta;
    gm[3 * C + k] = sigma * sigma;
    gm[4 * C + k] = beta * beta;
}

int gm_scratch_doubles() { return kGmBlocks * kGmMaxC * 4; }

int est_gaussian_mixture(papof_handle* h, const double* im1, const double* im2, int H, int W, int C, double* gm,
                         double* scratch) {
    if (C > kGmMaxC) return PAPOF_EINVAL;
    for (int it = 0; it < 3; it++) {
        hipLaunchKernelGGL(k_gm_partial, dim3(kGmBlocks), dim3(kGmThreads), 0, h->stream, im1, im2, (size_t)H * W, C, gm,
                           scratch);
        hipLaunchKernelGGL(k_gm_mstep, dim3(1), dim3(64), 0, h->stream, scratch, C, 0.9, gm);
    }
    LAUNCH_CHECK();
    return PAPOF_OK;
}

constexpr int kLapBlocks = 256, kLapThreads = 256, kLapMaxC = 8;
static __global__ __launch_bounds__(kLapThreads) void k_lap_partial(const double* __restrict__ im1,
                                                             const double* __restrict__ im2,
                                                             const double* __restrict__ u, const double* __restrict__ v,
                                                             int H, int W, int C, double* __restrict__ partial) {
    __shared__ double red[kLapThreads];
    const size_t np = (size_t)H * W;
    double acc[kLapMaxC][2];
    for (int k = 0; k < kLapMaxC; k++) acc[k][0] = acc[k][1] = 0.0;
    for (size_t o = (size_t)blockIdx.x * kLapThreads + threadIdx.x; o < np; o += (size_t)kLapBlocks * kLapThreads) {
        const int i = (int)(o / W), j = (int)(o - (size_t)i * W);
        const double fu = u ? u[o] : 0.0, fv = u ? v[o] : 0.0;
#pragma unroll
        for (int k = 0; k < kLapMaxC; k++) {
            if (k >= C) break;
            const double w = u ? warp_value(im1 + k * np, im2 + k * np, fu, fv, i, j, H, W) : im2[k * np + o];
            const double d = fabs(im1[k * np + o] - w);
            if (lap_valid(d)) {
                acc[k][0] += d;
                acc[k][1] += 1.0;
            }
        }
    }
    for (int k = 0; k < C; k++)
        for (int q = 0; q < 2; q++) {
            red[threadIdx.x] = acc[k][q];
            __syncthreads();
            for (int s = kLapThreads / 2; s > 0; s >>= 1) {
                if ((int)threadIdx.x < s) red[threadIdx.x] += red[threadIdx.x + s];
                __syncthreads();
            }
            if (threadIdx.x == 0) partial[((size_t)blockIdx.x * kLapMaxC + k) * 2 + q] = red[0];
            __syncthreads();
        }
}
static __global__ void k_lap_finish(const double* __restrict__ partial, int C, double* __restrict__ lap) {
    const int k = threadIdx.x;
    if (k >= C) return;
    double s = 0.0, n = 0.0;
    for (int b = 0; b < kLapBlocks; b++) {
        s += partial[((size_t)b * kLapMaxC + k) * 2];
        n += partial[((size_t)b * kLapMaxC + k) * 2 + 1];
    }
    lap[k] = n == 0 ? 0.001 : s / n;
}
static __global__ __launch_bounds__(256) void k_lap_small(const double* __restrict__ im1, const double* __restrict__ im2,
                                                       const double* __restrict__ u, const double* __restrict__ v, int H,
                                                       int W, unsigned* __restrict__ wit, double wit_thr, unsigned mark,
                                                       BatchK bk) {
    const int np = H * W;
    {
        const size_t p = blockIdx.y;
        batch_frames(bk, p, im1, im2);
        u += p * bk.uv;
        v += p * bk.uv;
        wit += p * bk.wit;
    }
    const double *p1 = im1 + (size_t)blockIdx.x * np, *p2 = im2 + (size_t)blockIdx.x * np;
    bool hit = false, valid = false;
    for (int o = threadIdx.x; o < np; o += 256) {
        const int i = o / W, j = o - i * W;
        const double d = fabs(p1[o] - warp_value(p1, p2, u[o], v[o], i, j, H, W));
        valid = valid || lap_valid(d);
        hit = hit || lap_witness(d, wit_thr);
    }
    const int any_hit = __syncthreads_or(hit ? 1 : 0), any_valid = __syncthreads_or(valid ? 1 : 0);
    if (threadIdx.x == 0 && (any_hit || !any_valid)) wit[blockIdx.x] = any_hit ? mark : (mark ^ kLapNone);
}
static __global__ __launch_bounds__(256) void k_lap_rows(const double* __restrict__ im1, const double* __restrict__ im2,
                                                      const double* __restrict__ u, const double* __restrict__ v, int H,
                                                      int W, int r0, int r1, unsigned* __restrict__ wit,
                                                      unsigned* __restrict__ val, double wit_thr, unsigned mark) {
    const size_t np = (size_t)H * W;
    const double *p1 = im1 + blockIdx.y * np, *p2 = im2 + blockIdx.y * np;
// ... 77 lines not shown
```

Before: 216.1.

## Fuse pyramid smoothing into resize and compute bicubic gradients inline

Adds a tiled LDS kernel that applies the separable Gaussian and the bilinear downsample in one pass, so most pyramid levels no longer write and reread full-size filtered temporaries. The final bicubic warp now computes the central-difference gradients (gx, gy, gxy) from a 4x4 neighbourhood inside the kernel, which removes the central3 precompute pass, its three planes, and the cross-stream wait on it. Temp buffers shrink to cover only levels that still use the unfused path. The trade-off is extra register pressure and redundant arithmetic in the warp kernel, plus LDS-capacity limits that decide which levels take the fused path.

New measurement: 219.4, median of 6. 1.02x the previous value.

```diff
diff --git a/papteam_opticalflow_amd/csrc/api.hip b/papteam_opticalflow_amd/csrc/api.hip
--- a/papteam_opticalflow_amd/csrc/api.hip
+++ b/papteam_opticalflow_amd/csrc/api.hip
@@ -47,7 +47,7 @@
     planes += (size_t)2 * C + 2 * C;
     planes += (size_t)7 * fc;
     planes += 8;
-    planes += (size_t)3 * C + C;
+    planes += (size_t)C;
     planes += (size_t)3 * fc;
     size_t bytes = planes * np * sizeof(double);
     bytes += 3 * (sor_cells + 2 * kLanes) * 16 + (sor_cells_d + 2 * kLanes) * 16 + 10 * np * sizeof(double);
@@ -173,12 +173,26 @@
     return PAPOF_OK;
 }
 
+static bool level_is_resize_only(const Taps& g) { return g.fsize == 0 && g.t[0] == 1.0; }
+static bool level_is_fused(const Taps& g, const PyrPlan& p, int dh, int dw) {
+    return smooth_resize_fits(g, g, p.sh, p.sw, dh, dw, p.rate, p.rate);
+}
 int smooth_and_resize(papof_handle* h, const double* src, double* dst, double* tmp_a, double* tmp_b, const PyrPlan& p, int C,
                       int dh, int dw) {
     const Taps g = gaussian_taps(p.sigma, p.fsize);
-    if (g.fsize == 0 && g.t[0] == 1.0) return resize(h, src, dst, p.sh, p.sw, C, dh, dw, p.rate, p.rate, false, 0.0);
+    if (level_is_resize_only(g)) return resize(h, src, dst, p.sh, p.sw, C, dh, dw, p.rate, p.rate, false, 0.0);
+    if (level_is_fused(g, p, dh, dw)) return smooth_resize(h, src, dst, p.sh, p.sw, C, dh, dw, p.rate, p.rate, g, g);
     PAPOF_TRY(filter_hv(h, src, tmp_b, tmp_a, p.sh, p.sw, C, g, g));
     return resize(h, tmp_b, dst, p.sh, p.sw, C, dh, dw, p.rate, p.rate, false, 0.0);
+}
+size_t pyramid_tmp_elems(const std::vector<Level>& L, const std::vector<PyrPlan>& plan, int C) {
+    size_t n = 0;
+    for (size_t i = 1; i < L.size(); i++) {
+        const Taps g = gaussian_taps(plan[i].sigma, plan[i].fsize);
+        if (!level_is_resize_only(g) && !level_is_fused(g, plan[i], L[i].h, L[i].w))
+            n = std::max(n, (size_t)plan[i].sw * plan[i].sh * C);
+    }
+    return n;
 }
 
 int reduce_init(papof_handle* h, const papof_tensor* a, const papof_tensor* b, int pairs_a, int pairs_b, int H, int W,
@@ -454,7 +468,6 @@
     int slot1 = 0;
     double *tmp_a = nullptr, *tmp_b = nullptr;
     std::vector<double*> F1, F2, S1;
-    double *gx = nullptr, *gy = nullptr, *gxy = nullptr;
     double *prep_tmp = nullptr, *warp = nullptr;
     double *u = nullptr, *v = nullptr, *u2 = nullptr, *v2 = nullptr;
     SolveBuffers B;
@@ -493,9 +506,9 @@
         l.p1 = slot[S.slot1];
         l.p2 = slot[S.slot1 ^ 1];
     }
-    const size_t np0 = (size_t)S.H * S.W;
-    S.tmp_a = A.f64(np0 * S.C);
-    S.tmp_b = A.f64(np0 * S.C);
+    const size_t tmp = pyramid_tmp_elems(S.cp.L, S.cp.plan, S.C);
+    S.tmp_a = A.f64(tmp);
+    S.tmp_b = A.f64(tmp);
     return A.overflow ? PAPOF_ENOMEM : PAPOF_OK;
 }
 
@@ -515,9 +528,6 @@
         S.S1[k] = A.f64(n);
     }
     S.prep_tmp = A.f64(np0 * fc);
-    S.gx = A.f64(np0 * S.C);
-    S.gy = A.f64(np0 * S.C);
-    S.gxy = A.f64(np0 * S.C);
     S.warp = A.f64(np0 * fc);
     S.u = A.f64(2 * np0);
     S.v = S.u ? S.u + np0 : nullptr;
@@ -573,11 +583,6 @@
     }
     return PAPOF_OK;
 }
-static int prep_final_planes(FlowPass& S) {
-    S.pclk.phase(PAPOF_T_POSTPROCESSING);
-    PAPOF_TRY(central3_planes(S.h, S.cp.L[0].p2, S.gx, S.gy, S.gxy, S.H, S.W, S.C));
-    return prep_level_ready(S, S.cp.levels);
-}
 static int prep_upload(FlowPass& S, const void* host, const FrameIn& f, int event) {
     papof_handle* h = S.h;
     if (!host) return PAPOF_OK;
@@ -601,7 +606,7 @@
         PAPOF_TRY(prep_upload(S, S.h->hostio.im2, S.fb, 1));
         PAPOF_TRY(prep_frames(S, 1, 2, chained, false, true));
     }
-    return prep_final_planes(S);
+    return PAPOF_OK;
 }
 
 static int fork_and_prepare(FlowPass& S) {
@@ -681,11 +686,9 @@
 static int final_warp(FlowPass& S) {
     papof_handle* h = S.h;
     papof_handle::HostIO& io = h->hostio;
-    const int H = S.H, W = S.W, C = S.C, levels = S.cp.levels;
+    const int H = S.H, W = S.W, C = S.C;
     const size_t np0 = (size_t)H * W;
     const Level& l0 = S.cp.L[0];
-    S.clk.phase(-1);
-    if (S.overlap) PAPOF_HIP(hipStreamWaitEvent(S.main_stream, h->sync_events[levels], 0));
     S.clk.phase(PAPOF_T_POSTPROCESSING);
     if (S.hostio && io.early_out && S.u == S.d_vx && S.v == S.d_vy) {
         hipStream_t const cs = h->copy_stream;
@@ -697,7 +700,7 @@
         for (int q = 0; q < kChunks; q++) {
             const Rect rc{0, (int)((long long)H * q / kChunks), W, (int)((long long)H * (q + 1) / kChunks)};
             if (rc.empty()) continue;
-            PAPOF_TRY(bicubic_warp(h, l0.p1, l0.p2, S.gx, S.gy, S.gxy, S.u, S.v, S.d_warp, H, W, C, &rc));
+            PAPOF_TRY(bicubic_warp(h, l0.p1, l0.p2, nullptr, nullptr, nullptr, S.u, S.v, S.d_warp, H, W, C, &rc));
             PAPOF_HIP(hipEventRecord(h->copy_events[3 + q], S.main_stream));
             PAPOF_HIP(hipStreamWaitEvent(cs, h->copy_events[3 + q], 0));
             const size_t off = (size_t)rc.y0 * W * C, cnt = (size_t)rc.h() * W * C;
@@ -706,7 +709,7 @@
         io.out_issued = true;
         return PAPOF_OK;
     }
-    PAPOF_TRY(bicubic_warp(h, l0.p1, l0.p2, S.gx, S.gy, S.gxy, S.u, S.v, S.d_warp, H, W, C));
+    PAPOF_TRY(bicubic_warp(h, l0.p1, l0.p2, nullptr, nullptr, nullptr, S.u, S.v, S.d_warp, H, W, C));
     if (S.u != S.d_vx) PAPOF_HIP(hipMemcpyAsync(S.d_vx, S.u, np0 * sizeof(double), hipMemcpyDeviceToDevice, h->stream));
     if (S.v != S.d_vy) PAPOF_HIP(hipMemcpyAsync(S.d_vy, S.v, np0 * sizeof(double), hipMemcpyDeviceToDevice, h->stream));
     return PAPOF_OK;
@@ -1666,17 +1669,16 @@
 int papof_stage_bicubic_warp_ex(papof_handle* h, const double* im1, const double* im2, const double* vx,
                                 const double* vy, int height, int width, int c, int clamp, double* out) {
     if (!h || !im1 || !im2 || !vx || !vy || !out || height < 1 || width < 1 || c < 1) return PAPOF_EINVAL;
-    Scope S(h, img_bytes(height, width, c, 10) + img_bytes(height, width, 1, 4));
+    Scope S(h, img_bytes(height, width, c, 7) + img_bytes(height, width, 1, 4));
     PAPOF_TRY(S.rc);
     const size_t n = (size_t)height * width * c;
     double* a = S.up_planar(im1, height, width, c);
     double* b = S.up_planar(im2, height, width, c);
     double* fx = S.up_planar(vx, height, width, 1);
     double* fy = S.up_planar(vy, height, width, 1);
-    double *gx = S.dev(n), *gy = S.dev(n), *gxy = S.dev(n), *o = S.dev(n);
-    PAPOF_TRY(S.rc);
-    PAPOF_TRY(central3_planes(h, b, gx, gy, gxy, height, width, c));
-    PAPOF_TRY(bicubic_warp(h, a, b, gx, gy, gxy, fx, fy, o, height, width, c, nullptr, false, clamp != 0));
+    double* o = S.dev(n);
+    PAPOF_TRY(S.rc);
+    PAPOF_TRY(bicubic_warp(h, a, b, nullptr, nullptr, nullptr, fx, fy, o, height, width, c, nullptr, false, clamp != 0));
     PAPOF_HIP(hipMemcpyAsync(out, o, n * sizeof(double), hipMemcpyDeviceToHost, h->stream));
     PAPOF_HIP(hipStreamSynchronize(h->stream));
     return PAPOF_OK;
diff --git a/papteam_opticalflow_amd/csrc/common.h b/papteam_opticalflow_amd/csrc/common.h
--- a/papteam_opticalflow_amd/csrc/common.h
+++ b/papteam_opticalflow_amd/csrc/common.h
@@ -290,6 +290,9 @@
            double yr, bool use_post, double post, const Rect* rc = nullptr);
 int im2feature(papof_handle* h, const double* im, double* feat, int H, int W, int C, unsigned* nz = nullptr, int frames = 1,
                size_t nz_stride = 0);
+bool smooth_resize_fits(const Taps& fh, const Taps& fv, int sh, int sw, int dh, int dw, double xr, double yr);
+int smooth_resize(papof_handle* h, const double* src, double* dst, int sh, int sw, int planes, int dh, int dw, double xr,
+                  double yr, const Taps& fh, const Taps& fv);
 int central3_planes(papof_handle* h, const double* src, double* gx, double* gy, double* gxy, int H, int W, int planes);
 int warp_bilinear(papof_handle* h, const double* im1, const double* im2, const double* vx, const double* vy,
                   double* out, int H, int W, int planes, const Rect* rc = nullptr);
diff --git a/papteam_opticalflow_amd/csrc/flow_internal.h b/papteam_opticalflow_amd/csrc/flow_internal.h
--- a/papteam_opticalflow_amd/csrc/flow_internal.h
+++ b/papteam_opticalflow_amd/csrc/flow_internal.h
@@ -170,6 +170,7 @@
 int pyramid_plan(int H, int W, double ratio, int nlev, std::vector<Level>& L, std::vector<PyrPlan>& plan);
 int build_pyramid(papof_handle* h, const std::vector<Level>& L, const std::vector<PyrPlan>& plan, int C, bool second,
                   double* tmp_a, double* tmp_b);
+size_t pyramid_tmp_elems(const std::vector<Level>& L, const std::vector<PyrPlan>& plan, int C);
 int smooth_and_resize(papof_handle* h, const double* src, double* dst, double* tmp_a, double* tmp_b, const PyrPlan& p, int C,
                       int dh, int dw);
 int feature_channels(int C);
diff --git a/papteam_opticalflow_amd/csrc/kernels.hip b/papteam_opticalflow_amd/csrc/kernels.hip
--- a/papteam_opticalflow_amd/csrc/kernels.hip
+++ b/papteam_opticalflow_amd/csrc/kernels.hip
@@ -20,7 +20,7 @@
 }
 __global__ void k_stamp(unsigned long long* s) { stamp_now(s); }
 
-__device__ __forceinline__ int clampi(int x, int n) {
+__host__ __device__ __forceinline__ int clampi(int x, int n) {
     x = x < 0 ? 0 : x;
     return x > n - 1 ? n - 1 : x;
 }
@@ -289,32 +289,48 @@
     int o[4];
     double s[4];
 };
+struct BilinearAxis {
+    int c[2];
+    double d;
+};
+
+__host__ __device__ __forceinline__ BilinearAxis bilinear_axis(int n, double x) {
+    BilinearAxis a;
+    const int xx = (int)x;
+    double dx = x - xx;
+    dx = dx > 1 ? 1.0 : dx;
+    dx = dx < 0 ? 0.0 : dx;
+    a.d = dx;
+    a.c[0] = clampi(xx, n);
+    a.c[1] = clampi(xx + 1, n);
+    return a;
+}
 
 __device__ __forceinline__ BilinearTaps bilinear_taps(int W, int H, double x, double y) {
     BilinearTaps b;
-    const int xx = (int)x, yy = (int)y;
-    double dx = x - xx, dy = y - yy;
-    dx = dx > 1 ? 1.0 : dx;
-    dx = dx < 0 ? 0.0 : dx;
-    dy = dy > 1 ? 1.0 : dy;
-    dy = dy < 0 ? 0.0 : dy;
+    const BilinearAxis ax = bilinear_axis(W, x), ay = bilinear_axis(H, y);
 #pragma unroll
     for (int m = 0; m <= 1; m++)
 #pragma unroll
         for (int n = 0; n <= 1; n++) {
-            const int u = clampi(xx + m, W), v = clampi(yy + n, H);
-            b.o[m * 2 + n] = v * W + u;
-            b.s[m * 2 + n] = fabs((double)(1 - m) - dx) * fabs((double)(1 - n) - dy);
+            b.o[m * 2 + n] = ay.c[n] * W + ax.c[m];
+            b.s[m * 2 + n] = fabs((double)(1 - m) - ax.d) * fabs((double)(1 - n) - ay.d);
         }
     return b;
 }
 
+template <class At>
+__device__ __forceinline__ double bilinear_sum(const BilinearTaps& b, At at) {
+    double acc = 0.0;
+#pragma unroll
+    for (int t = 0; t < 4; t++) acc += at(t) * b.s[t];
+    return acc;
+}
 __device__ __forceinline__ double bilinear_apply(const double* __restrict__ p, const BilinearTaps& b) {
-    double acc = 0.0;
-#pragma unroll
-    for (int t = 0; t < 4; t++) acc += p[b.o[t]] * b.s[t];
-    return acc;
-}
+    return bilinear_sum(b, [&](int t) { return p[b.o[t]]; });
+}
+
+__host__ __device__ __forceinline__ double resize_pos(int j, double r) { return (double)(j + 1) / r - 1; }
 
 __global__ void k_resize(const double* __restrict__ src, double* __restrict__ dst, int sh, int sw, int dh, int dw,
                          double xr, double yr, int use_post, double post, Rect rc, unsigned long long* stamp) {
@@ -323,12 +339,62 @@
     if (!xcd_tile((rc.x1 - rc.x0 + BX - 1) / BX, (rc.y1 - rc.y0 + BY - 1) / BY, tbx, tby)) return;
     const int j = rc.x0 + tbx * BX + threadIdx.x, i = rc.y0 + tby * BY + threadIdx.y;
     if (j >= rc.x1 || i >= rc.y1) return;
-    const double x = (double)(j + 1) / xr - 1;
-    const double y = (double)(i + 1) / yr - 1;
-    const BilinearTaps b = bilinear_taps(sw, sh, x, y);
+    const BilinearTaps b = bilinear_taps(sw, sh, resize_pos(j, xr), resize_pos(i, yr));
     double r = bilinear_apply(src + blockIdx.z * (size_t)sh * sw, b);
     if (use_post) r *= post;
     dst[blockIdx.z * (size_t)dh * dw + (size_t)i * dw + j] = r;
+}
+
+constexpr int kSrT = 16;
+template <int F>
+__global__ __launch_bounds__(256) void k_smooth_resize(const double* __restrict__ src, double* __restrict__ dst, int sh,
+                                                       int sw, int dh, int dw, double xr, double yr, Taps fh, Taps fv,
+                                                       int nx, int ny) {
+    extern __shared__ __align__(16) double sr_lds[];
+    int tx, ty;
+    if (!xcd_tile((dw + kSrT - 1) / kSrT, (dh + kSrT - 1) / kSrT, tx, ty)) return;
+    const int j0 = tx * kSrT, i0 = ty * kSrT;
+    const int j1 = min(j0 + kSrT, dw) - 1, i1 = min(i0 + kSrT, dh) - 1;
+    __shared__ double pos[2][kSrT];
+    const int t = threadIdx.y * BX + threadIdx.x;
+    if (t < kSrT)
+        pos[0][t] = resize_pos(j0 + t, xr);
+    else if (t < 2 * kSrT)
+        pos[1][t - kSrT] = resize_pos(i0 + t - kSrT, yr);
+    __syncthreads();
+    const int u_lo = bilinear_axis(sw, pos[0][0]).c[0], u_hi = bilinear_axis(sw, pos[0][j1 - j0]).c[1];
+    const int v_lo = bilinear_axis(sh, pos[1][0]).c[0], v_hi = bilinear_axis(sh, pos[1][i1 - i0]).c[1];
+    const int nxa = u_hi - u_lo + 1 + 2 * F, nya = v_hi - v_lo + 1 + 2 * F;
+    if (nxa > nx || nya > ny) return;
+    double* const raw = sr_lds;
+    double* const hs = sr_lds + (size_t)ny * nx;
+    const double* plane = src + blockIdx.z * (size_t)sh * sw;
+    for (int r = threadIdx.y; r < nya; r += BY) {
+        const double* row = plane + (size_t)clampi(v_lo - F + r, sh) * sw;
+        for (int c = threadIdx.x; c < nxa; c += BX) raw[r * nx + c] = row[clampi(u_lo - F + c, sw)];
+    }
+    __syncthreads();
+    {
+        const int slot = t % (2 * kSrT), m = slot / kSrT, jj = j0 + slot % kSrT;
+        if (jj <= j1) {
+            const BilinearAxis ax = bilinear_axis(sw, pos[0][jj - j0]);
+            const int cu = (m == 0 ? ax.c[0] : ax.c[1]) - u_lo + F;
+            for (int r = t / (2 * kSrT); r < nya; r += BX * BY / (2 * kSrT)) {
+                const double* at = raw + r * nx + cu;
+                hs[r * (2 * kSrT) + slot] = tap_sum<F>(fh, [&](int l) { return at[l]; });
+            }
+        }
+    }
+    __syncthreads();
+    const int ox = t % kSrT, j = j0 + ox, i = i0 + t / kSrT;
+    if (j > j1 || i > i1) return;
+    const double x = pos[0][j - j0], y = pos[1][i - i0];
+    const BilinearAxis ay = bilinear_axis(sh, y);
+    const BilinearTaps b = bilinear_taps(sw, sh, x, y);
+    dst[blockIdx.z * (size_t)dh * dw + (size_t)i * dw + j] = bilinear_sum(b, [&](int k) {
+        const double* at = hs + (ay.c[k % 2] - v_lo + F) * (2 * kSrT) + (k / 2) * kSrT + ox;
+        return tap_sum<F>(fv, [&](int l) { return at[l * (2 * kSrT)]; });
+    });
 }
 
 template <int C>
@@ -415,6 +481,19 @@
     }
 }
 
+template <class At>
+__device__ __forceinline__ double central3_h(const Taps& c3, At at) {
+    return tap_sum<1>(c3, [&](int l) { return at(0, l); });
+}
+template <class At>
+__device__ __forceinline__ double central3_v(const Taps& c3, At at) {
+    return tap_sum<1>(c3, [&](int l) { return at(l, 0); });
+}
+template <class HRow>
+__device__ __forceinline__ double central3_hv(const Taps& c3, HRow hrow) {
+    return tap_sum<1>(c3, [&](int l) { return hrow(l); });
+}
+
 __global__ void k_central3_all(const double* __restrict__ src, double* __restrict__ gx, double* __restrict__ gy,
                                double* __restrict__ gxy, int H, int W, Taps c3) {
     int tbx, tby;
@@ -423,23 +502,11 @@
     if (j >= W || i >= H) return;
     const size_t np = (size_t)H * W;
     const double* p = src + blockIdx.z * np;
-    const auto hrow = [&](int ii) {
-        const double* row = p + (size_t)ii * W;
-        double acc = 0.0;
-#pragma unroll
-        for (int l = -1; l <= 1; l++) acc += row[clampi(j + l, W)] * c3.t[l + 1];
-        return acc;
-    };
-    const double hx[3] = {hrow(clampi(i - 1, H)), hrow(i), hrow(clampi(i + 1, H))};
-    double vy = 0.0, vxy = 0.0;
-#pragma unroll
-    for (int l = -1; l <= 1; l++) vy += p[(size_t)clampi(i + l, H) * W + j] * c3.t[l + 1];
-#pragma unroll
-    for (int l = -1; l <= 1; l++) vxy += hx[l + 1] * c3.t[l + 1];
+    const auto at = [&](int dr, int dc) { return p[(size_t)clampi(i + dr, H) * W + clampi(j + dc, W)]; };
     const size_t o = blockIdx.z * np + (size_t)i * W + j;
-    gx[o] = hx[1];
-    gy[o] = vy;
-    gxy[o] = vxy;
+    gx[o] = central3_h(c3, at);
+    gy[o] = central3_v(c3, at);
+    gxy[o] = central3_hv(c3, [&](int l) { return central3_h(c3, [&](int, int dc) { return at(l, dc); }); });
 }
 
 __device__ __forceinline__ void warp_pixel(const double* __restrict__ im1, const double* __restrict__ im2,
@@ -1362,12 +1429,13 @@
     if (do_warp) warp_pixel(im1, im2, warp, fu, fv, i, j, H, W, planes);
 }
 
-template <bool BATCH>
-__global__ void k_bicubic(const double* __restrict__ im1, const double* __restrict__ im2,
-                          const double* __restrict__ gx, const double* __restrict__ gy,
-                          const double* __restrict__ gxy, const double* __restrict__ vx,
-                          const double* __restrict__ vy, double* __restrict__ out, int H, int W, int C, Rect rc,
-                          unsigned long long* stamp, int planar_out, int clamp, BatchK bk) {
+template <bool BATCH, bool GRAD, int CC = -1>
+__device__ __forceinline__ void bicubic_pixel(const double* __restrict__ im1, const double* __restrict__ im2,
+                                              const double* __restrict__ gx, const double* __restrict__ gy,
+                                              const double* __restrict__ gxy, const Taps& c3, const double* __restrict__ vx,
+                                              const double* __restrict__ vy, double* __restrict__ out, int H, int W, int C,
+                                              const Rect& rc, unsigned long long* stamp, int planar_out, int clamp,
+                                              const BatchK& bk) {
     if (BATCH) {
         const size_t p = blockIdx.y;
         const ptrdiff_t o1 = (ptrdiff_t)batch_frames(bk, p, im1, im2);
@@ -1409,12 +1477,50 @@
     const double dx2 = dx * dx, dy2 = dy * dy;
     const double dx3 = dx * dx2, dy3 = dy * dy2;
     const size_t a = (size_t)y0 * W + x0, b = (size_t)y0 * W + x1, c = (size_t)y1 * W + x0, d = (size_t)y1 * W + x1;
-    for (int k = 0; k < C; k++) {
-        const double *f = im2 + k * np, *px = gx + k * np, *py = gy + k * np, *pz = gxy + k * np;
-        const double fA = f[a], fB = f[b], fC = f[c], fD = f[d];
-        const double xA = px[a], xB = px[b], xC = px[c], xD = px[d];
-        const double yA = py[a], yB = py[b], yC = py[c], yD = py[d];
-        const double zA = pz[a], zB = pz[b], zC = pz[c], zD = pz[d];
+    size_t ro[4], co[4];
+    if (GRAD) {
+        ro[0] = (size_t)clampi(y0 - 1, H) * W, ro[1] = (size_t)y0 * W, ro[2] = (size_t)y1 * W, ro[3] = (size_t)clampi(y1 + 1, H) * W;
+        co[0] = clampi(x0 - 1, W), co[1] = x0, co[2] = x1, co[3] = clampi(x1 + 1, W);
+    }
+    const auto nb = [](int corner, int d) { return corner == 0 ? 1 + d : (d == -1 ? 4 : 2 + d); };
+    const int nc = CC > 0 ? CC : C;
+#pragma unroll
+    for (int k = 0; k < nc; k++) {
+        const double* f = im2 + k * np;
+        double fA, fB, fC, fD, xA, xB, xC, xD, yA, yB, yC, yD, zA, zB, zC, zD;
+        if (GRAD) {
+            double e[5][4], h[5][2];
+#pragma unroll
+            for (int r = 0; r < 4; r++)
+#pragma unroll
+                for (int q = 0; q < 4; q++) e[r][q] = f[ro[r] + co[q]];
+#pragma unroll
+            for (int r = 0; r < 4; r++) {
+                const double left1 = x1 != x0 ? e[r][1] : e[r][0];
+                h[r][0] = central3_h(c3, [&](int, int dc) { return e[r][1 + dc]; });
+                h[r][1] = central3_h(c3, [&](int, int dc) { return dc == -1 ? left1 : e[r][2 + dc]; });
+            }
+#pragma unroll
+            for (int q = 1; q <= 2; q++) e[4][q] = y1 != y0 ? e[1][q] : e[0][q];
+#pragma unroll
+            for (int cx = 0; cx < 2; cx++) h[4][cx] = y1 != y0 ? h[1][cx] : h[0][cx];
+            const auto corner = [&](int cy, int cx, double& fv, double& dxv, double& dyv, double& dxyv) {
+                fv = e[1 + cy][1 + cx];
+                dxv = h[1 + cy][cx];
+                dyv = central3_v(c3, [&](int dr, int) { return e[nb(cy, dr)][1 + cx]; });
+                dxyv = central3_hv(c3, [&](int l) { return h[nb(cy, l)][cx]; });
+            };
+            corner(0, 0, fA, xA, yA, zA);
+            corner(0, 1, fB, xB, yB, zB);
+            corner(1, 0, fC, xC, yC, zC);
+            corner(1, 1, fD, xD, yD, zD);
+        } else {
+            const double *px = gx + k * np, *py = gy + k * np, *pz = gxy + k * np;
+            fA = f[a], fB = f[b], fC = f[c], fD = f[d];
+            xA = px[a], xB = px[b], xC = px[c], xD = px[d];
+            yA = py[a], yB = py[b], yC = py[c], yD = py[d];
+            zA = pz[a], zB = pz[b], zC = pz[c], zD = pz[d];
+        }
         const double c00 = fA;
         const double c10 = xA;
         const double c20 = -3 * fA + 3 * fB - 2 * xA - xB;
@@ -1446,6 +1552,29 @@
     }
 }
 
+template <bool BATCH>
+__global__ void k_bicubic(const double* __restrict__ im1, const double* __restrict__ im2,
+                          const double* __restrict__ gx, const double* __restrict__ gy,
+                          const double* __restrict__ gxy, const double* __restrict__ vx,
+                          const double* __restrict__ vy, double* __restrict__ out, int H, int W, int C, Rect rc,
+                          unsigned long long* stamp, int planar_out, int clamp, BatchK bk) {
+    bicubic_pixel<BATCH, false>(im1, im2, gx, gy, gxy, Taps{}, vx, vy, out, H, W, C, rc, stamp, planar_out, clamp, bk);
+}
+
+__global__ void k_bicubic_grad(const double* __restrict__ im1, const double* __restrict__ im2, Taps c3,
+                               const double* __restrict__ vx, const double* __restrict__ vy, double* __restrict__ out, int H,
+                               int W, int C, Rect rc, unsigned long long* stamp, int planar_out, int clamp) {
+    bicubic_pixel<false, true, -1>(im1, im2, nullptr, nullptr, nullptr, c3, vx, vy, out, H, W, C, rc, stamp, planar_out, clamp,
+                                   BatchK{});
+}
+__global__ __attribute__((amdgpu_waves_per_eu(5, 5))) void k_bicubic_grad3(
+    const double* __restrict__ im1, const double* __restrict__ im2, Taps c3, const double* __restrict__ vx,
+    const double* __restrict__ vy, double* __restrict__ out, int H, int W, int C, Rect rc, unsigned long long* stamp,
+    int planar_out, int clamp) {
+    bicubic_pixel<false, true, 3>(im1, im2, nullptr, nullptr, nullptr, c3, vx, vy, out, H, W, C, rc, stamp, planar_out, clamp,
+                                  BatchK{});
+}
+
 __global__ void k_flow_quantize16(const double* __restrict__ vx, const double* __restrict__ vy,
                                   unsigned short* __restrict__ q, size_t n) {
     const size_t i = (size_t)blockIdx.x * blockDim.x + threadIdx.x;
@@ -1726,6 +1855,60 @@
     if (r.empty()) return PAPOF_OK;
     hipLaunchKernelGGL(k_resize, dim3(xcd_grid(tiles_of(r.x1 - r.x0, BX), tiles_of(r.y1 - r.y0, BY)), 1, planes), dim3(BX, BY), 0, h->stream, src, dst, sh, sw, dh, dw, xr, yr,
                        use_post ? 1 : 0, post, r, take_stamp(h));
+    LAUNCH_CHECK();
+    return PAPOF_OK;
+}
+
+namespace {
+constexpr size_t kSrMaxLds = 64 * 1024;
+struct SrShape {
+    int nx, ny;
+    size_t lds;
+};
+SrShape sr_shape(int f, int sh, int sw, int dh, int dw, double xr, double yr) {
+    const auto span = [](int n_src, int n_dst, double r) {
+        int s = 0;
+        for (int p0 = 0; p0 < n_dst; p0 += kSrT)
+            s = std::max(s, bilinear_axis(n_src, resize_pos(std::min(p0 + kSrT, n_dst) - 1, r)).c[1] -
+                                bilinear_axis(n_src, resize_pos(p0, r)).c[0] + 1);
+        return s;
+    };
+    SrShape s;
+    s.nx = (span(sw, dw, xr) + 2 * f) | 1;
+    s.ny = span(sh, dh, yr) + 2 * f;
+    s.lds = ((size_t)s.ny * s.nx + (size_t)s.ny * 2 * kSrT) * sizeof(double);
+    return s;
+}
+}
+
+bool smooth_resize_fits(const Taps& fh, const Taps& fv, int sh, int sw, int dh, int dw, double xr, double yr) {
+    if (fh.fsize != fv.fsize || fh.fsize < 1 || fh.fsize > kHvMaxF || dh < 1 || dw < 1 || !(xr > 0) || !(yr > 0)) return false;
+    return sr_shape(fh.fsize, sh, sw, dh, dw, xr, yr).lds <= kSrMaxLds;
+}
+
+int smooth_resize(papof_handle* h, const double* src, double* dst, int sh, int sw, int planes, int dh, int dw, double xr,
+                  double yr, const Taps& fh, const Taps& fv) {
+    if (!smooth_resize_fits(fh, fv, sh, sw, dh, dw, xr, yr)) return PAPOF_EINVAL;
+    const SrShape s = sr_shape(fh.fsize, sh, sw, dh, dw, xr, yr);
+    const dim3 grid(xcd_grid(tiles_of(dw, kSrT), tiles_of(dh, kSrT)), 1, planes), block(BX, BY);
+#define PAPOF_SR(FF)                                                                                                        \
+    do {                                                                                                                    \
+        static bool attr_set = false;                    \
+        if (!attr_set) {                                                                                                    \
+            PAPOF_HIP(hipFuncSetAttribute((const void*)k_smooth_resize<FF>, hipFuncAttributeMaxDynamicSharedMemorySize,     \
+                                          (int)kSrMaxLds));                                                                 \
+            attr_set = true;                                                                                                \
+        }                                                                                                                   \
+        hipLaunchKernelGGL(k_smooth_resize<FF>, grid, block, s.lds, h->stream, src, dst, sh, sw, dh, dw, xr, yr, fh, fv,    \
+                           s.nx, s.ny);                                                                                     \
+    } while (0)
+    switch (fh.fsize) {
+        case 1: PAPOF_SR(1); break;
+        case 2: PAPOF_SR(2); break;
+        case 3: PAPOF_SR(3); break;
+        default: PAPOF_SR(4); break;
+    }
+#undef PAPOF_SR
     LAUNCH_CHECK();
     return PAPOF_OK;
 }
@@ -1915,6 +2098,13 @@
                  const Rect* rc, bool planar_out, bool clamp, int batch, const BatchK* bk) {
     const Rect r = region(rc, W, H);
     if (r.empty()) return PAPOF_OK;
+    if (!gx) {
+        if (gy || gxy || batch > 1) return PAPOF_EINVAL;
+        hipLaunchKernelGGL(C == 3 ? k_bicubic_grad3 : k_bicubic_grad, dim3(xcd_grid(tiles_of(r.x1 - r.x0, BX), tiles_of(r.y1 - r.y0, BY))), dim3(BX, BY), 0, h->stream, im1, im2,
+                           central3_taps(), vx, vy, out_hwc, H, W, C, r, take_stamp(h), planar_out ? 1 : 0, clamp ? 1 : 0);
+        LAUNCH_CHECK();
+        return PAPOF_OK;
+    }
     hipLaunchKernelGGL(batch > 1 ? k_bicubic<true> : k_bicubic<false>, dim3(xcd_grid(tiles_of(r.x1 - r.x0, BX), tiles_of(r.y1 - r.y0, BY)), batch), dim3(BX, BY), 0, h->stream, im1, im2, gx, gy, gxy, vx, vy, out_hwc, H, W,
                        C, r, take_stamp(h), planar_out ? 1 : 0, clamp ? 1 : 0, bk ? *bk : kNoBatch);
     LAUNCH_CHECK();
```
